# avadakadabra0909/geth-sharding

Hardware: AMD Instinct MI355X
Metric: ecrecover sigs/sec + Keccak collation GB/s (higher is better)
Workload: dtype u32; 1 GPU; 1M-signature secp256k1 ecrecover + Keccak-256 address derivation per GPU (BASELINE.json configs[1]); signatures_per_gpu=1048576, parallelism=shard-partitioned x1, batches_in_flight=2

## Files before the change

geth-sharding_amd/csrc/fe9_asm.cuh:

```cuda
#pragma once
#include <stdint.h>
namespace gsv {
__device__ __forceinline__ void fe9_mul_full(uint32_t r[9], const uint32_t a[9], const uint32_t b[9]) {
    uint64_t sd;
    uint32_t k31264 = 31264u, k256 = 256u, k977 = 977u, k8192 = 8192u;
    asm("v_mad_u64_u32 v[2:3], %9, %11, %27, 0\n\tv_mad_u64_u32 v[2:3], %9, %12, %26, v[2:3]\n\tv_mad_u64_u32 v[2:3], %9, %13, %25, v[2:3]\n\tv_mad_u64_u32 v[2:3], %9, %14, %24, v[2:3]\n\tv_mad_u64_u32 v[2:3], %9, %15, %23, v[2:3]\n\tv_mad_u64_u32 v[2:3], %9, %16, %22, v[2:3]\n\tv_mad_u64_u32 v[2:3], %9, %17, %21, v[2:3]\n\tv_mad_u64_u32 v[2:3], %9, %18, %20, v[2:3]\n\tv_mad_u64_u32 v[6:7], %9, v3, 8, 0\n\tv_mad_u64_u32 v[6:7], %9, %12, %27, v[6:7]\n\tv_mad_u64_u32 v[6:7], %9, %13, %26, v[6:7]\n\tv_mad_u64_u32 v[6:7], %9, %14, %25, v[6:7]\n\tv_mad_u64_u32 v[6:7], %9, %15, %24, v[6:7]\n\tv_mad_u64_u32 v[6:7], %9, %16, %23, v[6:7]\n\tv_mad_u64_u32 v[6:7], %9, %17, %22, v[6:7]\n\tv_mad_u64_u32 v[6:7], %9, %18, %21, v[6:7]\n\tv_mad_u64_u32 v[8:9], %9, v7, 8, 0\n\tv_mad_u64_u32 v[8:9], %9, %13, %27, v[8:9]\n\tv_mad_u64_u32 v[8:9], %9, %14, %26, v[8:9]\n\tv_mad_u64_u32 v[8:9], %9, %15, %25, v[8:9]\n\tv_mad_u64_u32 v[8:9], %9, %16, %24, v[8:9]\n\tv_mad_u64_u32 v[8:9], %9, %17, %23, v[8:9]\n\tv_mad_u64_u32 v[8:9], %9, %18, %22, v[8:9]\n\tv_mad_u64_u32 v[10:11], %9, v9, 8, 0\n\tv_mad_u64_u32 v[10:11], %9, %14, %27, v[10:11]\n\tv_mad_u64_u32 v[10:11], %9, %15, %26, v[10:11]\n\tv_mad_u64_u32 v[10:11], %9, %16, %25, v[10:11]\n\tv_mad_u64_u32 v[10:11], %9, %17, %24, v[10:11]\n\tv_mad_u64_u32 v[10:11], %9, %18, %23, v[10:11]\n\tv_mad_u64_u32 v[12:13], %9, v11, 8, 0\n\tv_mad_u64_u32 v[12:13], %9, %15, %27, v[12:13]\n\tv_mad_u64_u32 v[12:13], %9, %16, %26, v[12:13]\n\tv_mad_u64_u32 v[12:13], %9, %17, %25, v[12:13]\n\tv_mad_u64_u32 v[12:13], %9, %18, %24, v[12:13]\n\tv_mad_u64_u32 v[14:15], %9, v13, 8, 0\n\tv_mad_u64_u32 v[14:15], %9, %16, %27, v[14:15]\n\tv_mad_u64_u32 v[14:15], %9, %17, %26, v[14:15]\n\tv_mad_u64_u32 v[14:15], %9, %18, %25, v[14:15]\n\tv_mad_u64_u32 v[16:17], %9, v15, 8, 0\n\tv_mad_u64_u32 v[16:17], %9, %17, %27, v[16:17]\n\tv_mad_u64_u32 v[16:17], %9, %18, %26, v[16:17]\n\tv_mad_u64_u32 v[18:19], %9, v17, 8, 0\n\tv_mad_u64_u32 v[18:19], %9, %18, %27, v[18:19]\n\tv_lshlrev_b32 v3, 3, v19\n\tv_mad_u64_u32 v[4:5], %9, %10, %19, 0\n\tv_mad_u64_u32 v[4:5], %9, v2, %28, v[4:5]\n\tv_and_b32_e32 %0, 0x1fffffff, v4\n\tv_lshrrev_b64 v[4:5], 29, v[4:5]\n\tv_mad_u64_u32 v[4:5], %9, %10, %20, v[4:5]\n\tv_mad_u64_u32 v[4:5], %9, %11, %19, v[4:5]\n\tv_mad_u64_u32 v[4:5], %9, v6, %28, v[4:5]\n\tv_mad_u64_u32 v[4:5], %9, v2, %29, v[4:5]\n\tv_and_b32_e32 %1, 0x1fffffff, v4\n\tv_lshrrev_b64 v[4:5], 29, v[4:5]\n\tv_mad_u64_u32 v[4:5], %9, %10, %21, v[4:5]\n\tv_mad_u64_u32 v[4:5], %9, %11, %20, v[4:5]\n\tv_mad_u64_u32 v[4:5], %9, %12, %19, v[4:5]\n\tv_mad_u64_u32 v[4:5], %9, v8, %28, v[4:5]\n\tv_mad_u64_u32 v[4:5], %9, v6, %29, v[4:5]\n\tv_and_b32_e32 %2, 0x1fffffff, v4\n\tv_lshrrev_b64 v[4:5], 29, v[4:5]\n\tv_mad_u64_u32 v[4:5], %9, %10, %22, v[4:5]\n\tv_mad_u64_u32 v[4:5], %9, %11, %21, v[4:5]\n\tv_mad_u64_u32 v[4:5], %9, %12, %20, v[4:5]\n\tv_mad_u64_u32 v[4:5], %9, %13, %19, v[4:5]\n\tv_mad_u64_u32 v[4:5], %9, v10, %28, v[4:5]\n\tv_mad_u64_u32 v[4:5], %9, v8, %29, v[4:5]\n\tv_and_b32_e32 %3, 0x1fffffff, v4\n\tv_lshrrev_b64 v[4:5], 29, v[4:5]\n\tv_mad_u64_u32 v[4:5], %9, %10, %23, v[4:5]\n\tv_mad_u64_u32 v[4:5], %9, %11, %22, v[4:5]\n\tv_mad_u64_u32 v[4:5], %9, %12, %21, v[4:5]\n\tv_mad_u64_u32 v[4:5], %9, %13, %20, v[4:5]\n\tv_mad_u64_u32 v[4:5], %9, %14, %19, v[4:5]\n\tv_mad_u64_u32 v[4:5], %9, v12, %28, v[4:5]\n\tv_mad_u64_u32 v[4:5], %9, v10, %29, v[4:5]\n\tv_and_b32_e32 %4, 0x1fffffff, v4\n\tv_lshrrev_b64 v[4:5], 29, v[4:5]\n\tv_mad_u64_u32 v[4:5], %9, %10, %24, v[4:5]\n\tv_mad_u64_u32 v[4:5], %9, %11, %23, v[4:5]\n\tv_mad_u64_u32 v[4:5], %9, %12, %22, v[4:5]\n\tv_mad_u64_u32 v[4:5], %9, %13, %21, v[4:5]\n\tv_mad_u64_u32 v[4:5], %9, %14, %20, v[4:5]\n\tv_mad_u64_u32 v[4:5], %9, %15, %19, v[4:5]\n\tv_mad_u64_u32 v[4:5], %9, v14, %28, v[4:5]\n\tv_mad_u64_u32 v[4:5], %9, v12, %29, v[4:5]\n\tv_and_b32_e32 %5, 0x1fffffff, v4\n\tv_lshrrev_b64 v[4:5], 29, v[4:5]\n\tv_mad_u64_u32 v[4:5], %9, %10, %25, v[4:5]\n\tv_mad_u64_u32 v[4:5], %9, %11, %24, v[4:5]\n\tv_mad_u64_u32 v[4:5], %9, %12, %23, v[4:5]\n\tv_mad_u64_u32 v[4:5], %9, %13, %22, v[4:5]\n\tv_mad_u64_u32 v[4:5], %9, %14, %21, v[4:5]\n\tv_mad_u64_u32 v[4:5], %9, %15, %20, v[4:5]\n\tv_mad_u64_u32 v[4:5], %9, %16, %19, v[4:5]\n\tv_mad_u64_u32 v[4:5], %9, v16, %28, v[4:5]\n\tv_mad_u64_u32 v[4:5], %9, v14, %29, v[4:5]\n\tv_and_b32_e32 %6, 0x1fffffff, v4\n\tv_lshrrev_b64 v[4:5], 29, v[4:5]\n\tv_mad_u64_u32 v[4:5], %9, %10, %26, v[4:5]\n\tv_mad_u64_u32 v[4:5], %9, %11, %25, v[4:5]\n\tv_mad_u64_u32 v[4:5], %9, %12, %24, v[4:5]\n\tv_mad_u64_u32 v[4:5], %9, %13, %23, v[4:5]\n\tv_mad_u64_u32 v[4:5], %9, %14, %22, v[4:5]\n\tv_mad_u64_u32 v[4:5], %9, %15, %21, v[4:5]\n\tv_mad_u64_u32 v[4:5], %9, %16, %20, v[4:5]\n\tv_mad_u64_u32 v[4:5], %9, %17, %19, v[4:5]\n\tv_mad_u64_u32 v[4:5], %9, v18, %28, v[4:5]\n\tv_mad_u64_u32 v[4:5], %9, v16, %29, v[4:5]\n\tv_and_b32_e32 %7, 0x1fffffff, v4\n\tv_lshrrev_b64 v[4:5], 29, v[4:5]\n\tv_mad_u64_u32 v[4:5], %9, %10, %27, v[4:5]\n\tv_mad_u64_u32 v[4:5], %9, %11, %26, v[4:5]\n\tv_mad_u64_u32 v[4:5], %9, %12, %25, v[4:5]\n\tv_mad_u64_u32 v[4:5], %9, %13, %24, v[4:5]\n\tv_mad_u64_u32 v[4:5], %9, %14, %23, v[4:5]\n\tv_mad_u64_u32 v[4:5], %9, %15, %22, v[4:5]\n\tv_mad_u64_u32 v[4:5], %9, %16, %21, v[4:5]\n\tv_mad_u64_u32 v[4:5], %9, %17, %20, v[4:5]\n\tv_mad_u64_u32 v[4:5], %9, %18, %19, v[4:5]\n\tv_mad_u64_u32 v[4:5], %9, v3, %28, v[4:5]\n\tv_mad_u64_u32 v[4:5], %9, v18, %29, v[4:5]\n\tv_and_b32_e32 %8, 0xffffff, v4\n\tv_lshrrev_b64 v[4:5], 24, v[4:5]\n\tv_mad_u64_u32 v[6:7], %9, v3, %31, v[4:5]\n\tv_mov_b32 v5, 0\n\tv_mov_b32 v4, %0\n\tv_mad_u64_u32 v[4:5], %9, v6, %30, v[4:5]\n\tv_mad_u32_u24 v5, v7, %30, v5\n\tv_and_b32_e32 %0, 0x1fffffff, v4\n\tv_lshrrev_b64 v[4:5], 29, v[4:5]\n\tv_lshl_add_u64 v[4:5], v[6:7], 3, v[4:5]\n\tv_mad_u64_u32 v[4:5], %9, %1, 1, v[4:5]\n\tv_and_b32_e32 %1, 0x1fffffff, v4\n\tv_alignbit_b32 v6, v5, v4, 29\n\tv_add_u32 %2, %2, v6"
        : "=&v"(r[0]), "=&v"(r[1]), "=&v"(r[2]), "=&v"(r[3]), "=&v"(r[4]), "=&v"(r[5]), "=&v"(r[6]), "=&v"(r[7]), "=&v"(r[8]), "=&s"(sd)
        : "v"(a[0]), "v"(a[1]), "v"(a[2]), "v"(a[3]), "v"(a[4]), "v"(a[5]), "v"(a[6]), "v"(a[7]), "v"(a[8]), "v"(b[0]), "v"(b[1]), "v"(b[2]), "v"(b[3]), "v"(b[4]), "v"(b[5]), "v"(b[6]), "v"(b[7]), "v"(b[8]), "s"(k31264), "s"(k256), "s"(k977), "s"(k8192)
        : "v2", "v3", "v4", "v5", "v6", "v7", "v8", "v9", "v10", "v11", "v12", "v13", "v14", "v15", "v16", "v17", "v18", "v19");
}
__device__ __forceinline__ void fe9_sqr_full(uint32_t r[9], const uint32_t a[9], const uint32_t b[9]) {
    uint64_t sd;
    uint32_t k31264 = 31264u, k256 = 256u, k977 = 977u, k8192 = 8192u;
    asm("v_mad_u64_u32 v[2:3], %9, %11, %27, 0\n\tv_mad_u64_u32 v[2:3], %9, %12, %26, v[2:3]\n\tv_mad_u64_u32 v[2:3], %9, %13, %25, v[2:3]\n\tv_mad_u64_u32 v[2:3], %9, %14, %24, v[2:3]\n\tv_mad_u64_u32 v[6:7], %9, v3, 8, 0\n\tv_mad_u64_u32 v[6:7], %9, %12, %27, v[6:7]\n\tv_mad_u64_u32 v[6:7], %9, %13, %26, v[6:7]\n\tv_mad_u64_u32 v[6:7], %9, %14, %25, v[6:7]\n\tv_mad_u64_u32 v[6:7], %9, %15, %15, v[6:7]\n\tv_mad_u64_u32 v[8:9], %9, v7, 8, 0\n\tv_mad_u64_u32 v[8:9], %9, %13, %27, v[8:9]\n\tv_mad_u64_u32 v[8:9], %9, %14, %26, v[8:9]\n\tv_mad_u64_u32 v[8:9], %9, %15, %25, v[8:9]\n\tv_mad_u64_u32 v[10:11], %9, v9, 8, 0\n\tv_mad_u64_u32 v[10:11], %9, %14, %27, v[10:11]\n\tv_mad_u64_u32 v[10:11], %9, %15, %26, v[10:11]\n\tv_mad_u64_u32 v[10:11], %9, %16, %16, v[10:11]\n\tv_mad_u64_u32 v[12:13], %9, v11, 8, 0\n\tv_mad_u64_u32 v[12:13], %9, %15, %27, v[12:13]\n\tv_mad_u64_u32 v[12:13], %9, %16, %26, v[12:13]\n\tv_mad_u64_u32 v[14:15], %9, v13, 8, 0\n\tv_mad_u64_u32 v[14:15], %9, %16, %27, v[14:15]\n\tv_mad_u64_u32 v[14:15], %9, %17, %17, v[14:15]\n\tv_mad_u64_u32 v[16:17], %9, v15, 8, 0\n\tv_mad_u64_u32 v[16:17], %9, %17, %27, v[16:17]\n\tv_mad_u64_u32 v[18:19], %9, v17, 8, 0\n\tv_mad_u64_u32 v[18:19], %9, %18, %18, v[18:19]\n\tv_lshlrev_b32 v3, 3, v19\n\tv_mad_u64_u32 v[4:5], %9, %10, %10, 0\n\tv_mad_u64_u32 v[4:5], %9, v2, %28, v[4:5]\n\tv_and_b32_e32 %0, 0x1fffffff, v4\n\tv_lshrrev_b64 v[4:5], 29, v[4:5]\n\tv_mad_u64_u32 v[4:5], %9, %10, %20, v[4:5]\n\tv_mad_u64_u32 v[4:5], %9, v6, %28, v[4:5]\n\tv_mad_u64_u32 v[4:5], %9, v2, %29, v[4:5]\n\tv_and_b32_e32 %1, 0x1fffffff, v4\n\tv_lshrrev_b64 v[4:5], 29, v[4:5]\n\tv_mad_u64_u32 v[4:5], %9, %10, %21, v[4:5]\n\tv_mad_u64_u32 v[4:5], %9, %11, %11, v[4:5]\n\tv_mad_u64_u32 v[4:5], %9, v8, %28, v[4:5]\n\tv_mad_u64_u32 v[4:5], %9, v6, %29, v[4:5]\n\tv_and_b32_e32 %2, 0x1fffffff, v4\n\tv_lshrrev_b64 v[4:5], 29, v[4:5]\n\tv_mad_u64_u32 v[4:5], %9, %10, %22, v[4:5]\n\tv_mad_u64_u32 v[4:5], %9, %11, %21, v[4:5]\n\tv_mad_u64_u32 v[4:5], %9, v10, %28, v[4:5]\n\tv_mad_u64_u32 v[4:5], %9, v8, %29, v[4:5]\n\tv_and_b32_e32 %3, 0x1fffffff, v4\n\tv_lshrrev_b64 v[4:5], 29, v[4:5]\n\tv_mad_u64_u32 v[4:5], %9, %10, %23, v[4:5]\n\tv_mad_u64_u32 v[4:5], %9, %11, %22, v[4:5]\n\tv_mad_u64_u32 v[4:5], %9, %12, %12, v[4:5]\n\tv_mad_u64_u32 v[4:5], %9, v12, %28, v[4:5]\n\tv_mad_u64_u32 v[4:5], %9, v10, %29, v[4:5]\n\tv_and_b32_e32 %4, 0x1fffffff, v4\n\tv_lshrrev_b64 v[4:5], 29, v[4:5]\n\tv_mad_u64_u32 v[4:5], %9, %10, %24, v[4:5]\n\tv_mad_u64_u32 v[4:5], %9, %11, %23, v[4:5]\n\tv_mad_u64_u32 v[4:5], %9, %12, %22, v[4:5]\n\tv_mad_u64_u32 v[4:5], %9, v14, %28, v[4:5]\n\tv_mad_u64_u32 v[4:5], %9, v12, %29, v[4:5]\n\tv_and_b32_e32 %5, 0x1fffffff, v4\n\tv_lshrrev_b64 v[4:5], 29, v[4:5]\n\tv_mad_u64_u32 v[4:5], %9, %10, %25, v[4:5]\n\tv_mad_u64_u32 v[4:5], %9, %11, %24, v[4:5]\n\tv_mad_u64_u32 v[4:5], %9, %12, %23, v[4:5]\n\tv_mad_u64_u32 v[4:5], %9, %13, %13, v[4:5]\n\tv_mad_u64_u32 v[4:5], %9, v16, %28, v[4:5]\n\tv_mad_u64_u32 v[4:5], %9, v14, %29, v[4:5]\n\tv_and_b32_e32 %6, 0x1fffffff, v4\n\tv_lshrrev_b64 v[4:5], 29, v[4:5]\n\tv_mad_u64_u32 v[4:5], %9, %10, %26, v[4:5]\n\tv_mad_u64_u32 v[4:5], %9, %11, %25, v[4:5]\n\tv_mad_u64_u32 v[4:5], %9, %12, %24, v[4:5]\n\tv_mad_u64_u32 v[4:5], %9, %13, %23, v[4:5]\n\tv_mad_u64_u32 v[4:5], %9, v18, %28, v[4:5]\n\tv_mad_u64_u32 v[4:5], %9, v16, %29, v[4:5]\n\tv_and_b32_e32 %7, 0x1fffffff, v4\n\tv_lshrrev_b64 v[4:5], 29, v[4:5]\n\tv_mad_u64_u32 v[4:5], %9, %10, %27, v[4:5]\n\tv_mad_u64_u32 v[4:5], %9, %11, %26, v[4:5]\n\tv_mad_u64_u32 v[4:5], %9, %12, %25, v[4:5]\n\tv_mad_u64_u32 v[4:5], %9, %13, %24, v[4:5]\n\tv_mad_u64_u32 v[4:5], %9, %14, %14, v[4:5]\n\tv_mad_u64_u32 v[4:5], %9, v3, %28, v[4:5]\n\tv_mad_u64_u32 v[4:5], %9, v18, %29, v[4:5]\n\tv_and_b32_e32 %8, 0xffffff, v4\n\tv_lshrrev_b64 v[4:5], 24, v[4:5]\n\tv_mad_u64_u32 v[6:7], %9, v3, %31, v[4:5]\n\tv_mov_b32 v5, 0\n\tv_mov_b32 v4, %0\n\tv_mad_u64_u32 v[4:5], %9, v6, %30, v[4:5]\n\tv_mad_u32_u24 v5, v7, %30, v5\n\tv_and_b32_e32 %0, 0x1fffffff, v4\n\tv_lshrrev_b64 v[4:5], 29, v[4:5]\n\tv_lshl_add_u64 v[4:5], v[6:7], 3, v[4:5]\n\tv_mad_u64_u32 v[4:5], %9, %1, 1, v[4:5]\n\tv_and_b32_e32 %1, 0x1fffffff, v4\n\tv_alignbit_b32 v6, v5, v4, 29\n\tv_add_u32 %2, %2, v6"
        : "=&v"(r[0]), "=&v"(r[1]), "=&v"(r[2]), "=&v"(r[3]), "=&v"(r[4]), "=&v"(r[5]), "=&v"(r[6]), "=&v"(r[7]), "=&v"(r[8]), "=&s"(sd)
        : "v"(a[0]), "v"(a[1]), "v"(a[2]), "v"(a[3]), "v"(a[4]), "v"(a[5]), "v"(a[6]), "v"(a[7]), "v"(a[8]), "v"(b[0]), "v"(b[1]), "v"(b[2]), "v"(b[3]), "v"(b[4]), "v"(b[5]), "v"(b[6]), "v"(b[7]), "v"(b[8]), "s"(k31264), "s"(k256), "s"(k977), "s"(k8192)
        : "v2", "v3", "v4", "v5", "v6", "v7", "v8", "v9", "v10", "v11", "v12", "v13", "v14", "v15", "v16", "v17", "v18", "v19");
}
__device__ __forceinline__ void fe9_mul_add_full(uint32_t r[9], const uint32_t a[9], const uint32_t b[9], const uint32_t c[9]) {
    uint64_t sd;
    uint32_t k31264 = 31264u, k256 = 256u, k977 = 977u, k8192 = 8192u;
    asm("v_mad_u64_u32 v[2:3], %9, %11, %27, 0\n\tv_mad_u64_u32 v[2:3], %9, %12, %26, v[2:3]\n\tv_mad_u64_u32 v[2:3], %9, %13, %25, v[2:3]\n\tv_mad_u64_u32 v[2:3], %9, %14, %24, v[2:3]\n\tv_mad_u64_u32 v[2:3], %9, %15, %23, v[2:3]\n\tv_mad_u64_u32 v[2:3], %9, %16, %22, v[2:3]\n\tv_mad_u64_u32 v[2:3], %9, %17, %21, v[2:3]\n\tv_mad_u64_u32 v[2:3], %9, %18, %20, v[2:3]\n\tv_mad_u64_u32 v[6:7], %9, v3, 8, 0\n\tv_mad_u64_u32 v[6:7], %9, %12, %27, v[6:7]\n\tv_mad_u64_u32 v[6:7], %9, %13, %26, v[6:7]\n\tv_mad_u64_u32 v[6:7], %9, %14, %25, v[6:7]\n\tv_mad_u64_u32 v[6:7], %9, %15, %24, v[6:7]\n\tv_mad_u64_u32 v[6:7], %9, %16, %23, v[6:7]\n\tv_mad_u64_u32 v[6:7], %9, %17, %22, v[6:7]\n\tv_mad_u64_u32 v[6:7], %9, %18, %21, v[6:7]\n\tv_mad_u64_u32 v[8:9], %9, v7, 8, 0\n\tv_mad_u64_u32 v[8:9], %9, %13, %27, v[8:9]\n\tv_mad_u64_u32 v[8:9], %9, %14, %26, v[8:9]\n\tv_mad_u64_u32 v[8:9], %9, %15, %25, v[8:9]\n\tv_mad_u64_u32 v[8:9], %9, %16, %24, v[8:9]\n\tv_mad_u64_u32 v[8:9], %9, %17, %23, v[8:9]\n\tv_mad_u64_u32 v[8:9], %9, %18, %22, v[8:9]\n\tv_mad_u64_u32 v[10:11], %9, v9, 8, 0\n\tv_mad_u64_u32 v[10:11], %9, %14, %27, v[10:11]\n\tv_mad_u64_u32 v[10:11], %9, %15, %26, v[10:11]\n\tv_mad_u64_u32 v[10:11], %9, %16, %25, v[10:11]\n\tv_mad_u64_u32 v[10:11], %9, %17, %24, v[10:11]\n\tv_mad_u64_u32 v[10:11], %9, %18, %23, v[10:11]\n\tv_mad_u64_u32 v[12:13], %9, v11, 8, 0\n\tv_mad_u64_u32 v[12:13], %9, %15, %27, v[12:13]\n\tv_mad_u64_u32 v[12:13], %9, %16, %26, v[12:13]\n\tv_mad_u64_u32 v[12:13], %9, %17, %25, v[12:13]\n\tv_mad_u64_u32 v[12:13], %9, %18, %24, v[12:13]\n\tv_mad_u64_u32 v[14:15], %9, v13, 8, 0\n\tv_mad_u64_u32 v[14:15], %9, %16, %27, v[14:15]\n\tv_mad_u64_u32 v[14:15], %9, %17, %26, v[14:15]\n\tv_mad_u64_u32 v[14:15], %9, %18, %25, v[14:15]\n\tv_mad_u64_u32 v[16:17], %9, v15, 8, 0\n\tv_mad_u64_u32 v[16:17], %9, %17, %27, v[16:17]\n\tv_mad_u64_u32 v[16:17], %9, %18, %26, v[16:17]\n\tv_mad_u64_u32 v[18:19], %9, v17, 8, 0\n\tv_mad_u64_u32 v[18:19], %9, %18, %27, v[18:19]\n\tv_lshlrev_b32 v3, 3, v19\n\tv_mad_u64_u32 v[4:5], %9, %32, 1, 0\n\tv_mad_u64_u32 v[4:5], %9, %10, %19, v[4:5]\n\tv_mad_u64_u32 v[4:5], %9, v2, %28, v[4:5]\n\tv_and_b32_e32 %0, 0x1fffffff, v4\n\tv_lshrrev_b64 v[4:5], 29, v[4:5]\n\tv_mad_u64_u32 v[4:5], %9, %33, 1, v[4:5]\n\tv_mad_u64_u32 v[4:5], %9, %10, %20, v[4:5]\n\tv_mad_u64_u32 v[4:5], %9, %11, %19, v[4:5]\n\tv_mad_u64_u32 v[4:5], %9, v6, %28, v[4:5]\n\tv_mad_u64_u32 v[4:5], %9, v2, %29, v[4:5]\n\tv_and_b32_e32 %1, 0x1fffffff, v4\n\tv_lshrrev_b64 v[4:5], 29, v[4:5]\n\tv_mad_u64_u32 v[4:5], %9, %34, 1, v[4:5]\n\tv_mad_u64_u32 v[4:5], %9, %10, %21, v[4:5]\n\tv_mad_u64_u32 v[4:5], %9, %11, %20, v[4:5]\n\tv_mad_u64_u32 v[4:5], %9, %12, %19, v[4:5]\n\tv_mad_u64_u32 v[4:5], %9, v8, %28, v[4:5]\n\tv_mad_u64_u32 v[4:5], %9, v6, %29, v[4:5]\n\tv_and_b32_e32 %2, 0x1fffffff, v4\n\tv_lshrrev_b64 v[4:5], 29, v[4:5]\n\tv_mad_u64_u32 v[4:5], %9, %35, 1, v[4:5]\n\tv_mad_u64_u32 v[4:5], %9, %10, %22, v[4:5]\n\tv_mad_u64_u32 v[4:5], %9, %11, %21, v[4:5]\n\tv_mad_u64_u32 v[4:5], %9, %12, %20, v[4:5]\n\tv_mad_u64_u32 v[4:5], %9, %13, %19, v[4:5]\n\tv_mad_u64_u32 v[4:5], %9, v10, %28, v[4:5]\n\tv_mad_u64_u32 v[4:5], %9, v8, %29, v[4:5]\n\tv_and_b32_e32 %3, 0x1fffffff, v4\n\tv_lshrrev_b64 v[4:5], 29, v[4:5]\n\tv_mad_u64_u32 v[4:5], %9, %36, 1, v[4:5]\n\tv_mad_u64_u32 v[4:5], %9, %10, %23, v[4:5]\n\tv_mad_u64_u32 v[4:5], %9, %11, %22, v[4:5]\n\tv_mad_u64_u32 v[4:5], %9, %12, %21, v[4:5]\n\tv_mad_u64_u32 v[4:5], %9, %13, %20, v[4:5]\n\tv_mad_u64_u32 v[4:5], %9, %14, %19, v[4:5]\n\tv_mad_u64_u32 v[4:5], %9, v12, %28, v[4:5]\n\tv_mad_u64_u32 v[4:5], %9, v10, %29, v[4:5]\n\tv_and_b32_e32 %4, 0x1fffffff, v4\n\tv_lshrrev_b64 v[4:5], 29, v[4:5]\n\tv_mad_u64_u32 v[4:5], %9, %37, 1, v[4:5]\n\tv_mad_u64_u32 v[4:5], %9, %10, %24, v[4:5]\n\tv_mad_u64_u32 v[4:5], %9, %11, %23, v[4:5]\n\tv_mad_u64_u32 v[4:5], %9, %12, %22, v[4:5]\n\tv_mad_u64_u32 v[4:5], %9, %13, %21, v[4:5]\n\tv_mad_u64_u32 v[4:5], %9, %14, %20, v[4:5]\n\tv_mad_u64_u32 v[4:5], %9, %15, %19, v[4:5]\n\tv_mad_u64_u32 v[4:5], %9, v14, %28, v[4:5]\n\tv_mad_u64_u32 v[4:5], %9, v12, %29, v[4:5]\n\tv_and_b32_e32 %5, 0x1fffffff, v4\n\tv_lshrrev_b64 v[4:5], 29, v[4:5]\n\tv_mad_u64_u32 v[4:5], %9, %38, 1, v[4:5]\n\tv_mad_u64_u32 v[4:5], %9, %10, %25, v[4:5]\n\tv_mad_u64_u32 v[4:5], %9, %11, %24, v[4:5]\n\tv_mad_u64_u32 v[4:5], %9, %12, %23, v[4:5]\n\tv_mad_u64_u32 v[4:5], %9, %13, %22, v[4:5]\n\tv_mad_u64_u32 v[4:5], %9, %14, %21, v[4:5]\n\tv_mad_u64_u32 v[4:5], %9, %15, %20, v[4:5]\n\tv_mad_u64_u32 v[4:5], %9, %16, %19, v[4:5]\n\tv_mad_u64_u32 v[4:5], %9, v16, %28, v[4:5]\n\tv_mad_u64_u32 v[4:5], %9, v14, %29, v[4:5]\n\tv_and_b32_e32 %6, 0x1fffffff, v4\n\tv_lshrrev_b64 v[4:5], 29, v[4:5]\n\tv_mad_u64_u32 v[4:5], %9, %39, 1, v[4:5]\n\tv_mad_u64_u32 v[4:5], %9, %10, %26, v[4:5]\n\tv_mad_u64_u32 v[4:5], %9, %11, %25, v[4:5]\n\tv_mad_u64_u32 v[4:5], %9, %12, %24, v[4:5]\n\tv_mad_u64_u32 v[4:5], %9, %13, %23, v[4:5]\n\tv_mad_u64_u32 v[4:5], %9, %14, %22, v[4:5]\n\tv_mad_u64_u32 v[4:5], %9, %15, %21, v[4:5]\n\tv_mad_u64_u32 v[4:5], %9, %16, %20, v[4:5]\n\tv_mad_u64_u32 v[4:5], %9, %17, %19, v[4:5]\n\tv_mad_u64_u32 v[4:5], %9, v18, %28, v[4:5]\n\tv_mad_u64_u32 v[4:5], %9, v16, %29, v[4:5]\n\tv_and_b32_e32 %7, 0x1fffffff, v4\n\tv_lshrrev_b64 v[4:5], 29, v[4:5]\n\tv_mad_u64_u32 v[4:5], %9, %40, 1, v[4:5]\n\tv_mad_u64_u32 v[4:5], %9, %10, %27, v[4:5]\n\tv_mad_u64_u32 v[4:5], %9, %11, %26, v[4:5]\n\tv_mad_u64_u32 v[4:5], %9, %12, %25, v[4:5]\n\tv_mad_u64_u32 v[4:5], %9, %13, %24, v[4:5]\n\tv_mad_u64_u32 v[4:5], %9, %14, %23, v[4:5]\n\tv_mad_u64_u32 v[4:5], %9, %15, %22, v[4:5]\n\tv_mad_u64_u32 v[4:5], %9, %16, %21, v[4:5]\n\tv_mad_u64_u32 v[4:5], %9, %17, %20, v[4:5]\n\tv_mad_u64_u32 v[4:5], %9, %18, %19, v[4:5]\n\tv_mad_u64_u32 v[4:5], %9, v3, %28, v[4:5]\n\tv_mad_u64_u32 v[4:5], %9, v18, %29, v[4:5]\n\tv_and_b32_e32 %8, 0xffffff, v4\n\tv_lshrrev_b64 v[4:5], 24, v[4:5]\n\tv_mad_u64_u32 v[6:7], %9, v3, %31, v[4:5]\n\tv_mov_b32 v5, 0\n\tv_mov_b32 v4, %0\n\tv_mad_u64_u32 v[4:5], %9, v6, %30, v[4:5]\n\tv_mad_u32_u24 v5, v7, %30, v5\n\tv_and_b32_e32 %0, 0x1fffffff, v4\n\tv_lshrrev_b64 v[4:5], 29, v[4:5]\n\tv_lshl_add_u64 v[4:5], v[6:7], 3, v[4:5]\n\tv_mad_u64_u32 v[4:5], %9, %1, 1, v[4:5]\n\tv_and_b32_e32 %1, 0x1fffffff, v4\n\tv_alignbit_b32 v6, v5, v4, 29\n\tv_add_u32 %2, %2, v6"
        : "=&v"(r[0]), "=&v"(r[1]), "=&v"(r[2]), "=&v"(r[3]), "=&v"(r[4]), "=&v"(r[5]), "=&v"(r[6]), "=&v"(r[7]), "=&v"(r[8]), "=&s"(sd)
        : "v"(a[0]), "v"(a[1]), "v"(a[2]), "v"(a[3]), "v"(a[4]), "v"(a[5]), "v"(a[6]), "v"(a[7]), "v"(a[8]), "v"(b[0]), "v"(b[1]), "v"(b[2]), "v"(b[3]), "v"(b[4]), "v"(b[5]), "v"(b[6]), "v"(b[7]), "v"(b[8]), "s"(k31264), "s"(k256), "s"(k977), "s"(k8192), "v"(c[0]), "v"(c[1]), "v"(c[2]), "v"(c[3]), "v"(c[4]), "v"(c[5]), "v"(c[6]), "v"(c[7]), "v"(c[8])
        : "v2", "v3", "v4", "v5", "v6", "v7", "v8", "v9", "v10", "v11", "v12", "v13", "v14", "v15", "v16", "v17", "v18", "v19");
}
__device__ __forceinline__ void fe9_sqr_add_full(uint32_t r[9], const uint32_t a[9], const uint32_t b[9], const uint32_t c[9]) {
    uint64_t sd;
    uint32_t k31264 = 31264u, k256 = 256u, k977 = 977u, k8192 = 8192u;
    asm("v_mad_u64_u32 v[2:3], %9, %11, %27, 0\n\tv_mad_u64_u32 v[2:3], %9, %12, %26, v[2:3]\n\tv_mad_u64_u32 v[2:3], %9, %13, %25, v[2:3]\n\tv_mad_u64_u32 v[2:3], %9, %14, %24, v[2:3]\n\tv_mad_u64_u32 v[6:7], %9, v3, 8, 0\n\tv_mad_u64_u32 v[6:7], %9, %12, %27, v[6:7]\n\tv_mad_u64_u32 v[6:7], %9, %13, %26, v[6:7]\n\tv_mad_u64_u32 v[6:7], %9, %14, %25, v[6:7]\n\tv_mad_u64_u32 v[6:7], %9, %15, %15, v[6:7]\n\tv_mad_u64_u32 v[8:9], %9, v7, 8, 0\n\tv_mad_u64_u32 v[8:9], %9, %13, %27, v[8:9]\n\tv_mad_u64_u32 v[8:9], %9, %14, %26, v[8:9]\n\tv_mad_u64_u32 v[8:9], %9, %15, %25, v[8:9]\n\tv_mad_u64_u32 v[10:11], %9, v9, 8, 0\n\tv_mad_u64_u32 v[10:11], %9, %14, %27, v[10:11]\n\tv_mad_u64_u32 v[10:11], %9, %15, %26, v[10:11]\n\tv_mad_u64_u32 v[10:11], %9, %16, %16, v[10:11]\n\tv_mad_u64_u32 v[12:13], %9, v11, 8, 0\n\tv_mad_u64_u32 v[12:13], %9, %15, %27, v[12:13]\n\tv_mad_u64_u32 v[12:13], %9, %16, %26, v[12:13]\n\tv_mad_u64_u32 v[14:15], %9, v13, 8, 0\n\tv_mad_u64_u32 v[14:15], %9, %16, %27, v[14:15]\n\tv_mad_u64_u32 v[14:15], %9, %17, %17, v[14:15]\n\tv_mad_u64_u32 v[16:17], %9, v15, 8, 0\n\tv_mad_u64_u32 v[16:17], %9, %17, %27, v[16:17]\n\tv_mad_u64_u32 v[18:19], %9, v17, 8, 0\n\tv_mad_u64_u32 v[18:19], %9, %18, %18, v[18:19]\n\tv_lshlrev_b32 v3, 3, v19\n\tv_mad_u64_u32 v[4:5], %9, %32, 1, 0\n\tv_mad_u64_u32 v[4:5], %9, %10, %10, v[4:5]\n\tv_mad_u64_u32 v[4:5], %9, v2, %28, v[4:5]\n\tv_and_b32_e32 %0, 0x1fffffff, v4\n\tv_lshrrev_b64 v[4:5], 29, v[4:5]\n\tv_mad_u64_u32 v[4:5], %9, %33, 1, v[4:5]\n\tv_mad_u64_u32 v[4:5], %9, %10, %20, v[4:5]\n\tv_mad_u64_u32 v[4:5], %9, v6, %28, v[4:5]\n\tv_mad_u64_u32 v[4:5], %9, v2, %29, v[4:5]\n\tv_and_b32_e32 %1, 0x1fffffff, v4\n\tv_lshrrev_b64 v[4:5], 29, v[4:5]\n\tv_mad_u64_u32 v[4:5], %9, %34, 1, v[4:5]\n\tv_mad_u64_u32 v[4:5], %9, %10, %21, v[4:5]\n\tv_mad_u64_u32 v[4:5], %9, %11, %11, v[4:5]\n\tv_mad_u64_u32 v[4:5], %9, v8, %28, v[4:5]\n\tv_mad_u64_u32 v[4:5], %9, v6, %29, v[4:5]\n\tv_and_b32_e32 %2, 0x1fffffff, v4\n\tv_lshrrev_b64 v[4:5], 29, v[4:5]\n\tv_mad_u64_u32 v[4:5], %9, %35, 1, v[4:5]\n\tv_mad_u64_u32 v[4:5], %9, %10, %22, v[4:5]\n\tv_mad_u64_u32 v[4:5], %9, %11, %21, v[4:5]\n\tv_mad_u64_u32 v[4:5], %9, v10, %28, v[4:5]\n\tv_mad_u64_u32 v[4:5], %9, v8, %29, v[4:5]\n\tv_and_b32_e32 %3, 0x1fffffff, v4\n\tv_lshrrev_b64 v[4:5], 29, v[4:5]\n\tv_mad_u64_u32 v[4:5], %9, %36, 1, v[4:5]\n\tv_mad_u64_u32 v[4:5], %9, %10, %23, v[4:5]\n\tv_mad_u64_u32 v[4:5], %9, %11, %22, v[4:5]\n\tv_mad_u64_u32 v[4:5], %9, %12, %12, v[4:5]\n\tv_mad_u64_u32 v[4:5], %9, v12, %28, v[4:5]\n\tv_mad_u64_u32 v[4:5], %9, v10, %29, v[4:5]\n\tv_and_b32_e32 %4, 0x1fffffff, v4\n\tv_lshrrev_b64 v[4:5], 29, v[4:5]\n\tv_mad_u64_u32 v[4:5], %9, %37, 1, v[4:5]\n\tv_mad_u64_u32 v[4:5], %9, %10, %24, v[4:5]\n\tv_mad_u64_u32 v[4:5], %9, %11, %23, v[4:5]\n\tv_mad_u64_u32 v[4:5], %9, %12, %22, v[4:5]\n\tv_mad_u64_u32 v[4:5], %9, v14, %28, v[4:5]\n\tv_mad_u64_u32 v[4:5], %9, v12, %29, v[4:5]\n\tv_and_b32_e32 %5, 0x1fffffff, v4\n\tv_lshrrev_b64 v[4:5], 29, v[4:5]\n\tv_mad_u64_u32 v[4:5], %9, %38, 1, v[4:5]\n\tv_mad_u64_u32 v[4:5], %9, %10, %25, v[4:5]\n\tv_mad_u64_u32 v[4:5], %9, %11, %24, v[4:5]\n\tv_mad_u64_u32 v[4:5], %9, %12, %23, v[4:5]\n\tv_mad_u64_u32 v[4:5], %9, %13, %13, v[4:5]\n\tv_mad_u64_u32 v[4:5], %9, v16, %28, v[4:5]\n\tv_mad_u64_u32 v[4:5], %9, v14, %29, v[4:5]\n\tv_and_b32_e32 %6, 0x1fffffff, v4\n\tv_lshrrev_b64 v[4:5], 29, v[4:5]\n\tv_mad_u64_u32 v[4:5], %9, %39, 1, v[4:5]\n\tv_mad_u64_u32 v[4:5], %9, %10, %26, v[4:5]\n\tv_mad_u64_u32 v[4:5], %9, %11, %25, v[4:5]\n\tv_mad_u64_u32 v[4:5], %9, %12, %24, v[4:5]\n\tv_mad_u64_u32 v[4:5], %9, %13, %23, v[4:5]\n\tv_mad_u64_u32 v[4:5], %9, v18, %28, v[4:5]\n\tv_mad_u64_u32 v[4:5], %9, v16, %29, v[4:5]\n\tv_and_b32_e32 %7, 0x1fffffff, v4\n\tv_lshrrev_b64 v[4:5], 29, v[4:5]\n\tv_mad_u64_u32 v[4:5], %9, %40, 1, v[4:5]\n\tv_mad_u64_u32 v[4:5], %9, %10, %27, v[4:5]\n\tv_mad_u64_u32 v[4:5], %9, %11, %26, v[4:5]\n\tv_mad_u64_u32 v[4:5], %9, %12, %25, v[4:5]\n\tv_mad_u64_u32 v[4:5], %9, %13, %24, v[4:5]\n\tv_mad_u64_u32 v[4:5], %9, %14, %14, v[4:5]\n\tv_mad_u64_u32 v[4:5], %9, v3, %28, v[4:5]\n\tv_mad_u64_u32 v[4:5], %9, v18, %29, v[4:5]\n\tv_and_b32_e32 %8, 0xffffff, v4\n\tv_lshrrev_b64 v[4:5], 24, v[4:5]\n\tv_mad_u64_u32 v[6:7], %9, v3, %31, v[4:5]\n\tv_mov_b32 v5, 0\n\tv_mov_b32 v4, %0\n\tv_mad_u64_u32 v[4:5], %9, v6, %30, v[4:5]\n\tv_mad_u32_u24 v5, v7, %30, v5\n\tv_and_b32_e32 %0, 0x1fffffff, v4\n\tv_lshrrev_b64 v[4:5], 29, v[4:5]\n\tv_lshl_add_u64 v[4:5], v[6:7], 3, v[4:5]\n\tv_mad_u64_u32 v[4:5], %9, %1, 1, v[4:5]\n\tv_and_b32_e32 %1, 0x1fffffff, v4\n\tv_alignbit_b32 v6, v5, v4, 29\n\tv_add_u32 %2, %2, v6"
        : "=&v"(r[0]), "=&v"(r[1]), "=&v"(r[2]), "=&v"(r[3]), "=&v"(r[4]), "=&v"(r[5]), "=&v"(r[6]), "=&v"(r[7]), "=&v"(r[8]), "=&s"(sd)
        : "v"(a[0]), "v"(a[1]), "v"(a[2]), "v"(a[3]), "v"(a[4]), "v"(a[5]), "v"(a[6]), "v"(a[7]), "v"(a[8]), "v"(b[0]), "v"(b[1]), "v"(b[2]), "v"(b[3]), "v"(b[4]), "v"(b[5]), "v"(b[6]), "v"(b[7]), "v"(b[8]), "s"(k31264), "s"(k256), "s"(k977), "s"(k8192), "v"(c[0]), "v"(c[1]), "v"(c[2]), "v"(c[3]), "v"(c[4]), "v"(c[5]), "v"(c[6]), "v"(c[7]), "v"(c[8])
        : "v2", "v3", "v4", "v5", "v6", "v7", "v8", "v9", "v10", "v11", "v12", "v13", "v14", "v15", "v16", "v17", "v18", "v19");
}
__device__ __forceinline__ void fe9_dot_full(uint32_t r[9], const uint32_t a[9], const uint32_t b[9], const uint32_t c[9], const uint32_t d[9]) {
    uint64_t sd;
    uint32_t k31264 = 31264u, k256 = 256u, k977 = 977u, k8192 = 8192u;
    asm("v_mad_u64_u32 v[2:3], %9, %11, %27, 0\n\tv_mad_u64_u32 v[2:3], %9, %12, %26, v[2:3]\n\tv_mad_u64_u32 v[2:3], %9, %13, %25, v[2:3]\n\tv_mad_u64_u32 v[2:3], %9, %14, %24, v[2:3]\n\tv_mad_u64_u32 v[2:3], %9, %15, %23, v[2:3]\n\tv_mad_u64_u32 v[2:3], %9, %16, %22, v[2:3]\n\tv_mad_u64_u32 v[2:3], %9, %17, %21, v[2:3]\n\tv_mad_u64_u32 v[2:3], %9, %18, %20, v[2:3]\n\tv_mad_u64_u32 v[2:3], %9, %33, %49, v[2:3]\n\tv_mad_u64_u32 v[2:3], %9, %34, %48, v[2:3]\n\tv_mad_u64_u32 v[2:3], %9, %35, %47, v[2:3]\n\tv_mad_u64_u32 v[2:3], %9, %36, %46, v[2:3]\n\tv_mad_u64_u32 v[2:3], %9, %37, %45, v[2:3]\n\tv_mad_u64_u32 v[2:3], %9, %38, %44, v[2:3]\n\tv_mad_u64_u32 v[2:3], %9, %39, %43, v[2:3]\n\tv_mad_u64_u32 v[2:3], %9, %40, %42, v[2:3]\n\tv_mad_u64_u32 v[6:7], %9, v3, 8, 0\n\tv_mad_u64_u32 v[6:7], %9, %12, %27, v[6:7]\n\tv_mad_u64_u32 v[6:7], %9, %13, %26, v[6:7]\n\tv_mad_u64_u32 v[6:7], %9, %14, %25, v[6:7]\n\tv_mad_u64_u32 v[6:7], %9, %15, %24, v[6:7]\n\tv_mad_u64_u32 v[6:7], %9, %16, %23, v[6:7]\n\tv_mad_u64_u32 v[6:7], %9, %17, %22, v[6:7]\n\tv_mad_u64_u32 v[6:7], %9, %18, %21, v[6:7]\n\tv_mad_u64_u32 v[6:7], %9, %34, %49, v[6:7]\n\tv_mad_u64_u32 v[6:7], %9, %35, %48, v[6:7]\n\tv_mad_u64_u32 v[6:7], %9, %36, %47, v[6:7]\n\tv_mad_u64_u32 v[6:7], %9, %37, %46, v[6:7]\n\tv_mad_u64_u32 v[6:7], %9, %38, %45, v[6:7]\n\tv_mad_u64_u32 v[6:7], %9, %39, %44, v[6:7]\n\tv_mad_u64_u32 v[6:7], %9, %40, %43, v[6:7]\n\tv_mad_u64_u32 v[8:9], %9, v7, 8, 0\n\tv_mad_u64_u32 v[8:9], %9, %13, %27, v[8:9]\n\tv_mad_u64_u32 v[8:9], %9, %14, %26, v[8:9]\n\tv_mad_u64_u32 v[8:9], %9, %15, %25, v[8:9]\n\tv_mad_u64_u32 v[8:9], %9, %16, %24, v[8:9]\n\tv_mad_u64_u32 v[8:9], %9, %17, %23, v[8:9]\n\tv_mad_u64_u32 v[8:9], %9, %18, %22, v[8:9]\n\tv_mad_u64_u32 v[8:9], %9, %35, %49, v[8:9]\n\tv_mad_u64_u32 v[8:9], %9, %36, %48, v[8:9]\n\tv_mad_u64_u32 v[8:9], %9, %37, %47, v[8:9]\n\tv_mad_u64_u32 v[8:9], %9, %38, %46, v[8:9]\n\tv_mad_u64_u32 v[8:9], %9, %39, %45, v[8:9]\n\tv_mad_u64_u32 v[8:9], %9, %40, %44, v[8:9]\n\tv_mad_u64_u32 v[10:11], %9, v9, 8, 0\n\tv_mad_u64_u32 v[10:11], %9, %14, %27, v[10:11]\n\tv_mad_u64_u32 v[10:11], %9, %15, %26, v[10:11]\n\tv_mad_u64_u32 v[10:11], %9, %16, %25, v[10:11]\n\tv_mad_u64_u32 v[10:11], %9, %17, %24, v[10:11]\n\tv_mad_u64_u32 v[10:11], %9, %18, %23, v[10:11]\n\tv_mad_u64_u32 v[10:11], %9, %36, %49, v[10:11]\n\tv_mad_u64_u32 v[10:11], %9, %37, %48, v[10:11]\n\tv_mad_u64_u32 v[10:11], %9, %38, %47, v[10:11]\n\tv_mad_u64_u32 v[10:11], %9, %39, %46, v[10:11]\n\tv_mad_u64_u32 v[10:11], %9, %40, %45, v[10:11]\n\tv_mad_u64_u32 v[12:13], %9, v11, 8, 0\n\tv_mad_u64_u32 v[12:13], %9, %15, %27, v[12:13]\n\tv_mad_u64_u32 v[12:13], %9, %16, %26, v[12:13]\n\tv_mad_u64_u32 v[12:13], %9, %17, %25, v[12:13]\n\tv_mad_u64_u32 v[12:13], %9, %18, %24, v[12:13]\n\tv_mad_u64_u32 v[12:13], %9, %37, %49, v[12:13]\n\tv_mad_u64_u32 v[12:13], %9, %38, %48, v[12:13]\n\tv_mad_u64_u32 v[12:13], %9, %39, %47, v[12:13]\n\tv_mad_u64_u32 v[12:13], %9, %40, %46, v[12:13]\n\tv_mad_u64_u32 v[14:15], %9, v13, 8, 0\n\tv_mad_u64_u32 v[14:15], %9, %16, %27, v[14:15]\n\tv_mad_u64_u32 v[14:15], %9, %17, %26, v[14:15]\n\tv_mad_u64_u32 v[14:15], %9, %18, %25, v[14:15]\n\tv_mad_u64_u32 v[14:15], %9, %38, %49, v[14:15]\n\tv_mad_u64_u32 v[14:15], %9, %39, %48, v[14:15]\n\tv_mad_u64_u32 v[14:15], %9, %40, %47, v[14:15]\n\tv_mad_u64_u32 v[16:17], %9, v15, 8, 0\n\tv_mad_u64_u32 v[16:17], %9, %17, %27, v[16:17]\n\tv_mad_u64_u32 v[16:17], %9, %18, %26, v[16:17]\n\tv_mad_u64_u32 v[16:17], %9, %39, %49, v[16:17]\n\tv_mad_u64_u32 v[16:17], %9, %40, %48, v[16:17]\n\tv_mad_u64_u32 v[18:19], %9, v17, 8, 0\n\tv_mad_u64_u32 v[18:19], %9, %18, %27, v[18:19]\n\tv_mad_u64_u32 v[18:19], %9, %40, %49, v[18:19]\n\tv_lshlrev_b32 v3, 3, v19\n\tv_mad_u64_u32 v[4:5], %9, %10, %19, 0\n\tv_mad_u64_u32 v[4:5], %9, %32, %41, v[4:5]\n\tv_mad_u64_u32 v[4:5], %9, v2, %28, v[4:5]\n\tv_and_b32_e32 %0, 0x1fffffff, v4\n\tv_lshrrev_b64 v[4:5], 29, v[4:5]\n\tv_mad_u64_u32 v[4:5], %9, %10, %20, v[4:5]\n\tv_mad_u64_u32 v[4:5], %9, %11, %19, v[4:5]\n\tv_mad_u64_u32 v[4:5], %9, %32, %42, v[4:5]\n\tv_mad_u64_u32 v[4:5], %9, %33, %41, v[4:5]\n\tv_mad_u64_u32 v[4:5], %9, v6, %28, v[4:5]\n\tv_mad_u64_u32 v[4:5], %9, v2, %29, v[4:5]\n\tv_and_b32_e32 %1, 0x1fffffff, v4\n\tv_lshrrev_b64 v[4:5], 29, v[4:5]\n\tv_mad_u64_u32 v[4:5], %9, %10, %21, v[4:5]\n\tv_mad_u64_u32 v[4:5], %9, %11, %20, v[4:5]\n\tv_mad_u64_u32 v[4:5], %9, %12, %19, v[4:5]\n\tv_mad_u64_u32 v[4:5], %9, %32, %43, v[4:5]\n\tv_mad_u64_u32 v[4:5], %9, %33, %42, v[4:5]\n\tv_mad_u64_u32 v[4:5], %9, %34, %41, v[4:5]\n\tv_mad_u64_u32 v[4:5], %9, v8, %28, v[4:5]\n\tv_mad_u64_u32 v[4:5], %9, v6, %29, v[4:5]\n\tv_and_b32_e32 %2, 0x1fffffff, v4\n\tv_lshrrev_b64 v[4:5], 29, v[4:5]\n\tv_mad_u64_u32 v[4:5], %9, %10, %22, v[4:5]\n\tv_mad_u64_u32 v[4:5], %9, %11, %21, v[4:5]\n\tv_mad_u64_u32 v[4:5], %9, %12, %20, v[4:5]\n\tv_mad_u64_u32 v[4:5], %9, %13, %19, v[4:5]\n\tv_mad_u64_u32 v[4:5], %9, %32, %44, v[4:5]\n\tv_mad_u64_u32 v[4:5], %9, %33, %43, v[4:5]\n\tv_mad_u64_u32 v[4:5], %9, %34, %42, v[4:5]\n\tv_mad_u64_u32 v[4:5], %9, %35, %41, v[4:5]\n\tv_mad_u64_u32 v[4:5], %9, v10, %28, v[4:5]\n\tv_mad_u64_u32 v[4:5], %9, v8, %29, v[4:5]\n\tv_and_b32_e32 %3, 0x1fffffff, v4\n\tv_lshrrev_b64 v[4:5], 29, v[4:5]\n\tv_mad_u64_u32 v[4:5], %9, %10, %23, v[4:5]\n\tv_mad_u64_u32 v[4:5], %9, %11, %22, v[4:5]\n\tv_mad_u64_u32 v[4:5], %9, %12, %21, v[4:5]\n\tv_mad_u64_u32 v[4:5], %9, %13, %20, v[4:5]\n\tv_mad_u64_u32 v[4:5], %9, %14, %19, v[4:5]\n\tv_mad_u64_u32 v[4:5], %9, %32, %45, v[4:5]\n\tv_mad_u64_u32 v[4:5], %9, %33, %44, v[4:5]\n\tv_mad_u64_u32 v[4:5], %9, %34, %43, v[4:5]\n\tv_mad_u64_u32 v[4:5], %9, %35, %42, v[4:5]\n\tv_mad_u64_u32 v[4:5], %9, %36, %41, v[4:5]\n\tv_mad_u64_u32 v[4:5], %9, v12, %28, v[4:5]\n\tv_mad_u64_u32 v[4:5], %9, v10, %29, v[4:5]\n\tv_and_b32_e32 %4, 0x1fffffff, v4\n\tv_lshrrev_b64 v[4:5], 29, v[4:5]\n\tv_mad_u64_u32 v[4:5], %9, %10, %24, v[4:5]\n\tv_mad_u64_u32 v[4:5], %9, %11, %23, v[4:5]\n\tv_mad_u64_u32 v[4:5], %9, %12, %22, v[4:5]\n\tv_mad_u64_u32 v[4:5], %9, %13, %21, v[4:5]\n\tv_mad_u64_u32 v[4:5], %9, %14, %20, v[4:5]\n\tv_mad_u64_u32 v[4:5], %9, %15, %19, v[4:5]\n\tv_mad_u64_u32 v[4:5], %9, %32, %46, v[4:5]\n\tv_mad_u64_u32 v[4:5], %9, %33, %45, v[4:5]\n\tv_mad_u64_u32 v[4:5], %9, %34, %44, v[4:5]\n\tv_mad_u64_u32 v[4:5], %9, %35, %43, v[4:5]\n\tv_mad_u64_u32 v[4:5], %9, %36, %42, v[4:5]\n\tv_mad_u64_u32 v[4:5], %9, %37, %41, v[4:5]\n\tv_mad_u64_u32 v[4:5], %9, v14, %28, v[4:5]\n\tv_mad_u64_u32 v[4:5], %9, v12, %29, v[4:5]\n\tv_and_b32_e32 %5, 0x1fffffff, v4\n\tv_lshrrev_b64 v[4:5], 29, v[4:5]\n\tv_mad_u64_u32 v[4:5], %9, %10, %25, v[4:5]\n\tv_mad_u64_u32 v[4:5], %9, %11, %24, v[4:5]\n\tv_mad_u64_u32 v[4:5], %9, %12, %23, v[4:5]\n\tv_mad_u64_u32 v[4:5], %9, %13, %22, v[4:5]\n\tv_mad_u64_u32 v[4:5], %9, %14, %21, v[4:5]\n\tv_mad_u64_u32 v[4:5], %9, %15, %20, v[4:5]\n\tv_mad_u64_u32 v[4:5], %9, %16, %19, v[4:5]\n\tv_mad_u64_u32 v[4:5], %9, %32, %47, v[4:5]\n\tv_mad_u64_u32 v[4:5], %9, %33, %46, v[4:5]\n\tv_mad_u64_u32 v[4:5], %9, %34, %45, v[4:5]\n\tv_mad_u64_u32 v[4:5], %9, %35, %44, v[4:5]\n\tv_mad_u64_u32 v[4:5], %9, %36, %43, v[4:5]\n\tv_mad_u64_u32 v[4:5], %9, %37, %42, v[4:5]\n\tv_mad_u64_u32 v[4:5], %9, %38, %41, v[4:5]\n\tv_mad_u64_u32 v[4:5], %9, v16, %28, v[4:5]\n\tv_mad_u64_u32 v[4:5], %9, v14, %29, v[4:5]\n\tv_and_b32_e32 %6, 0x1fffffff, v4\n\tv_lshrrev_b64 v[4:5], 29, v[4:5]\n\tv_mad_u64_u32 v[4:5], %9, %10, %26, v[4:5]\n\tv_mad_u64_u32 v[4:5], %9, %11, %25, v[4:5]\n\tv_mad_u64_u32 v[4:5], %9, %12, %24, v[4:5]\n\tv_mad_u64_u32 v[4:5], %9, %13, %23, v[4:5]\n\tv_mad_u64_u32 v[4:5], %9, %14, %22, v[4:5]\n\tv_mad_u64_u32 v[4:5], %9, %15, %21, v[4:5]\n\tv_mad_u64_u32 v[4:5], %9, %16, %20, v[4:5]\n\tv_mad_u64_u32 v[4:5], %9, %17, %19, v[4:5]\n\tv_mad_u64_u32 v[4:5], %9, %32, %48, v[4:5]\n\tv_mad_u64_u32 v[4:5], %9, %33, %47, v[4:5]\n\tv_mad_u64_u32 v[4:5], %9, %34, %46, v[4:5]\n\tv_mad_u64_u32 v[4:5], %9, %35, %45, v[4:5]\n\tv_mad_u64_u32 v[4:5], %9, %36, %44, v[4:5]\n\tv_mad_u64_u32 v[4:5], %9, %37, %43, v[4:5]\n\tv_mad_u64_u32 v[4:5], %9, %38, %42, v[4:5]\n\tv_mad_u64_u32 v[4:5], %9, %39, %41, v[4:5]\n\tv_mad_u64_u32 v[4:5], %9, v18, %28, v[4:5]\n\tv_mad_u64_u32 v[4:5], %9, v16, %29, v[4:5]\n\tv_and_b32_e32 %7, 0x1fffffff, v4\n\tv_lshrrev_b64 v[4:5], 29, v[4:5]\n\tv_mad_u64_u32 v[4:5], %9, %10, %27, v[4:5]\n\tv_mad_u64_u32 v[4:5], %9, %11, %26, v[4:5]\n\tv_mad_u64_u32 v[4:5], %9, %12, %25, v[4:5]\n\tv_mad_u64_u32 v[4:5], %9, %13, %24, v[4:5]\n\tv_mad_u64_u32 v[4:5], %9, %14, %23, v[4:5]\n\tv_mad_u64_u32 v[4:5], %9, %15, %22, v[4:5]\n\tv_mad_u64_u32 v[4:5], %9, %16, %21, v[4:5]\n\tv_mad_u64_u32 v[4:5], %9, %17, %20, v[4:5]\n\tv_mad_u64_u32 v[4:5], %9, %18, %19, v[4:5]\n\tv_mad_u64_u32 v[4:5], %9, %32, %49, v[4:5]\n\tv_mad_u64_u32 v[4:5], %9, %33, %48, v[4:5]\n\tv_mad_u64_u32 v[4:5], %9, %34, %47, v[4:5]\n\tv_mad_u64_u32 v[4:5], %9, %35, %46, v[4:5]\n\tv_mad_u64_u32 v[4:5], %9, %36, %45, v[4:5]\n\tv_mad_u64_u32 v[4:5], %9, %37, %44, v[4:5]\n\tv_mad_u64_u32 v[4:5], %9, %38, %43, v[4:5]\n\tv_mad_u64_u32 v[4:5], %9, %39, %42, v[4:5]\n\tv_mad_u64_u32 v[4:5], %9, %40, %41, v[4:5]\n\tv_mad_u64_u32 v[4:5], %9, v3, %28, v[4:5]\n\tv_mad_u64_u32 v[4:5], %9, v18, %29, v[4:5]\n\tv_and_b32_e32 %8, 0xffffff, v4\n\tv_lshrrev_b64 v[4:5], 24, v[4:5]\n\tv_mad_u64_u32 v[6:7], %9, v3, %31, v[4:5]\n\tv_mov_b32 v5, 0\n\tv_mov_b32 v4, %0\n\tv_mad_u64_u32 v[4:5], %9, v6, %30, v[4:5]\n\tv_mad_u32_u24 v5, v7, %30, v5\n\tv_and_b32_e32 %0, 0x1fffffff, v4\n\tv_lshrrev_b64 v[4:5], 29, v[4:5]\n\tv_lshl_add_u64 v[4:5], v[6:7], 3, v[4:5]\n\tv_mad_u64_u32 v[4:5], %9, %1, 1, v[4:5]\n\tv_and_b32_e32 %1, 0x1fffffff, v4\n\tv_alignbit_b32 v6, v5, v4, 29\n\tv_add_u32 %2, %2, v6"
        : "=&v"(r[0]), "=&v"(r[1]), "=&v"(r[2]), "=&v"(r[3]), "=&v"(r[4]), "=&v"(r[5]), "=&v"(r[6]), "=&v"(r[7]), "=&v"(r[8]), "=&s"(sd)
        : "v"(a[0]), "v"(a[1]), "v"(a[2]), "v"(a[3]), "v"(a[4]), "v"(a[5]), "v"(a[6]), "v"(a[7]), "v"(a[8]), "v"(b[0]), "v"(b[1]), "v"(b[2]), "v"(b[3]), "v"(b[4]), "v"(b[5]), "v"(b[6]), "v"(b[7]), "v"(b[8]), "s"(k31264), "s"(k256), "s"(k977), "s"(k8192), "v"(c[0]), "v"(c[1]), "v"(c[2]), "v"(c[3]), "v"(c[4]), "v"(c[5]), "v"(c[6]), "v"(c[7]), "v"(c[8]), "v"(d[0]), "v"(d[1]), "v"(d[2]), "v"(d[3]), "v"(d[4]), "v"(d[5]), "v"(d[6]), "v"(d[7]), "v"(d[8])
        : "v2", "v3", "v4", "v5", "v6", "v7", "v8", "v9", "v10", "v11", "v12", "v13", "v14", "v15", "v16", "v17", "v18", "v19");
}
}
```

geth-sharding_amd/csrc/opcount.cuh:

```cuda
#pragma once

namespace gsv {
enum OpKind : int {
    OPC_FE_MUL = 0,
    OPC_FE_SQR = 1,
    OPC_SC_MUL = 2,
    OPC_SC_SQR = 3,
    OPC_BN_MUL = 4,
    OPC_MODINV = 5,
    OPC_BN_REDC = 6,
    OPC_FE_DOT = 7,
    OPC_N = 8
};
}

#if defined(GSV_OPCOUNT) && defined(__HIPCC__)
#include <hip/hip_runtime.h>
static __device__ unsigned long long gsv_opc_counts[gsv::OPC_N];
__device__ __forceinline__ void gsv_opc(int k) {
    unsigned long long m = __ballot(1);
    if ((int)__lane_id() == __ffsll((long long)m) - 1) atomicAdd(&gsv_opc_counts[k], (unsigned long long)__popcll(m));
}
#define GSV_OPC(k) gsv_opc(k)
#define GSV_OPCOUNT_READER(name)                                                                       \
    extern "C" int gsv_opcount_##name(unsigned long long* out, int reset) {                            \
        if (hipDeviceSynchronize() != hipSuccess) return -1;                                           \
        if (hipMemcpyFromSymbol(out, HIP_SYMBOL(gsv_opc_counts), sizeof(gsv_opc_counts)) != hipSuccess) \
            return -1;                                                                                 \
        if (reset) {                                                                                   \
            unsigned long long z[gsv::OPC_N] = {0};                                                    \
            if (hipMemcpyToSymbol(HIP_SYMBOL(gsv_opc_counts), z, sizeof(z)) != hipSuccess) return -1;  \
        }                                                                                              \
        return 0;                                                                                      \
    }
#else
#define GSV_OPC(k) ((void)0)
#define GSV_OPCOUNT_READER(name)
#endif
```

geth-sharding_amd/csrc/recover_dev.cuh:

```cuda
#pragma once
#include "gsv_internal.h"
#include "keccak_dev.cuh"
#include "secp256k1_dev.cuh"
namespace gsv { struct gej9; __device__ void gej9_dbl_rare(gej9& o, const gej9& p); }
#define GEJ9_DBL_RARE(o, p) gej9_dbl_rare(o, p)
#include "secp256k1_fe9.cuh"
#include "modinv30.cuh"

namespace gsv {

__device__ constexpr uint32_t BETA[8] = {0x719501EEu, 0xC1396C28u, 0x12F58995u, 0x9CF04975u,
                                         0xAC3434E9u, 0x6E64479Eu, 0x657C0710u, 0x7AE96A2Bu};
__device__ constexpr uint32_t MINUS_LAMBDA[8] = {0xB51283CFu, 0xE0CFC810u, 0x8EC739C2u, 0xA880B9FCu,
                                                 0x77ED9BA4u, 0x5AD9E3FDu, 0x3FA3CF1Fu, 0xAC9C52B3u};
__device__ constexpr uint32_t MINUS_B1[8] = {0x0ABFE4C3u, 0x6F547FA9u, 0x010E8828u, 0xE4437ED6u,
                                             0u, 0u, 0u, 0u};
__device__ constexpr uint32_t MINUS_B2[8] = {0x3DB1562Cu, 0xD765CDA8u, 0x0774346Du, 0x8A280AC5u,
                                             0xFFFFFFFEu, 0xFFFFFFFFu, 0xFFFFFFFFu, 0xFFFFFFFFu};
__device__ constexpr uint32_t GLV_G1[8] = {0xEB153DABu, 0x90E49284u, 0x6BCDE86Cu, 0xD221A7D4u,
                                           0x00003086u, 0u, 0u, 0u};
__device__ constexpr uint32_t GLV_G2[8] = {0xE4C42212u, 0x7FA90ABFu, 0x88286F54u, 0x7ED6010Eu,
                                           0x0000E443u, 0u, 0u, 0u};
__device__ constexpr uint32_t GX[8] = {0x16F81798u, 0x59F2815Bu, 0x2DCE28D9u, 0x029BFCDBu,
                                       0xCE870B07u, 0x55A06295u, 0xF9DCBBACu, 0x79BE667Eu};
__device__ constexpr uint32_t GY[8] = {0xFB10D4B8u, 0x9C47D08Fu, 0xA6855419u, 0xFD17B448u,
                                       0x0E1108A8u, 0x5DA4FBFCu, 0x26A3C465u, 0x483ADA77u};
__device__ constexpr uint32_t P_MINUS_N[8] = {0x2FC9BAEEu, 0x402DA172u, 0x50B75FC4u, 0x45512319u,
                                              0x00000001u, 0u, 0u, 0u};
__device__ constexpr uint32_t HALF_N[8] = {0x681B20A0u, 0xDFE92F46u, 0x57A4501Du, 0x5D576E73u,
                                           0xFFFFFFFFu, 0xFFFFFFFFu, 0xFFFFFFFFu, 0x7FFFFFFFu};

constexpr int GLV_W = 4;
constexpr int GLV_NT = 1 << (GLV_W - 1);
constexpr int GLV_DIGITS = (130 + GLV_W - 1) / GLV_W;
constexpr int DIG_SLOT = GLV_W <= 4 ? 4 : 8;
constexpr int DIG_PER_WORD = 32 / DIG_SLOT;
constexpr int DIG_WORDS = (GLV_DIGITS + DIG_PER_WORD - 1) / DIG_PER_WORD;
static_assert(GLV_W >= 3 && GLV_W <= 5, "GLV window width");
constexpr int GLV_LNT = 4;
static_assert(GLV_LNT <= GLV_NT, "LDS holds at most four entries at two waves per SIMD");
constexpr int GSV_LTAB_STRIDE = 256;
constexpr int GSV_LTAB_WORDS = 18 * GLV_LNT * GSV_LTAB_STRIDE;
#define GSV_ECR_WAVES 2
#define GSV_LTAB_DECL __shared__ uint32_t ltab[GSV_LTAB_WORDS]
#define GSV_LTAB_LANE (ltab + threadIdx.x)

GSV_DI void sc_from_const(sc& r, const uint32_t c[8]) {
#pragma unroll
    for (int i = 0; i < 8; i++) r.v[i] = c[i];
}

GSV_DI void sc_mul_shift272(sc& r, const sc& k, const uint32_t g[8]) {
    GSV_OPC(OPC_SC_MUL);
    uint32_t t[16];
    mul_8x8_fx(t, k.v, g);
#pragma unroll
    for (int i = 0; i < 7; i++) r.v[i] = (t[8 + i] >> 16) | (t[9 + i] << 16);
    r.v[7] = t[15] >> 16;
    uint64_t c = (uint64_t)r.v[0] + ((t[8] >> 15) & 1u);
    r.v[0] = lo32(c);
#pragma unroll
    for (int i = 1; i < 8; i++) {
        c = (uint64_t)r.v[i] + hi32(c);
        r.v[i] = lo32(c);
    }
}

GSV_DI void sc_split_lambda(sc& r1, sc& r2, const sc& k) {
    sc c1, c2, t;
    sc_mul_shift272(c1, k, GLV_G1);
    sc_mul_shift272(c2, k, GLV_G2);
    sc_from_const(t, MINUS_B1);
    sc_mul(c1, c1, t);
    sc_from_const(t, MINUS_B2);
    sc_mul(c2, c2, t);
    sc_add(r2, c1, c2);
    sc_from_const(t, MINUS_LAMBDA);
    sc_mul(r1, r2, t);
    sc_add(r1, r1, k);
}

GSV_DI bool sc_is_high(const sc& a) { return limbs_lt(HALF_N, a.v); }

GSV_DI void recode_glv(uint32_t dig[DIG_WORDS], uint32_t& skew, const sc& kin) {
    constexpr uint32_t MASK = (2u << GLV_W) - 1u;
    constexpr int32_t OFF = 1 << GLV_W;
    uint32_t k[5] = {kin.v[0], kin.v[1], kin.v[2], kin.v[3], kin.v[4]};
    skew = (k[0] & 1u) ^ 1u;
    uint64_t c = (uint64_t)k[0] + skew;
    k[0] = lo32(c);
#pragma unroll
    for (int i = 1; i < 5; i++) {
        c = (uint64_t)k[i] + hi32(c);
        k[i] = lo32(c);
    }
#pragma unroll
    for (int i = 0; i < DIG_WORDS; i++) dig[i] = 0;
#pragma unroll
    for (int i = 0; i < GLV_DIGITS; i++) {
        int32_t d;
        if (i < GLV_DIGITS - 1) d = (int32_t)(k[0] & MASK) - OFF;
        else d = (int32_t)(k[0] & MASK);
        uint32_t neg = d < 0 ? 1u : 0u;
        uint32_t mag = (uint32_t)(d < 0 ? -d : d);
        uint32_t code = (neg << (GLV_W - 1)) | ((mag - 1u) >> 1);
        dig[i / DIG_PER_WORD] |= code << ((i % DIG_PER_WORD) * DIG_SLOT);
        int64_t t = (int64_t)k[0] - d;
        uint32_t kk[5];
        kk[0] = (uint32_t)t;
        int64_t carry = t >> 32;
#pragma unroll
        for (int j = 1; j < 5; j++) {
            int64_t u = (int64_t)k[j] + carry;
            kk[j] = (uint32_t)u;
            carry = u >> 32;
        }
#pragma unroll
        for (int j = 0; j < 4; j++) k[j] = (kk[j] >> GLV_W) | (kk[j + 1] << (32 - GLV_W));
        k[4] = kk[4] >> GLV_W;
    }
}

GSV_DI void fe9_from_const(fe9& r, const uint32_t c[8]) {
    uint32_t w[8];
#pragma unroll
    for (int i = 0; i < 8; i++) w[i] = c[i];
    fe9_from_words(r, w);
}
GSV_DI void ge9_cmov(ge9& r, const ge9& a, bool f) {
    fe9_cmov(r.x, a.x, f);
    fe9_cmov(r.y, a.y, f);
}

typedef uint32_t gsv_v32 __attribute__((ext_vector_type(32)));
__device__ __noinline__ gsv_v32 gej9_dbl_ool(gsv_v32 in) {
    gej9 p, d;
#pragma unroll
    for (int i = 0; i < 9; i++) {
        p.x.v[i] = in[i];
        p.y.v[i] = in[9 + i];
        p.z.v[i] = in[18 + i];
    }
    gej9_dbl(d, p);
    gsv_v32 o;
#pragma unroll
    for (int i = 0; i < 9; i++) {
        o[i] = d.x.v[i];
        o[9 + i] = d.y.v[i];
        o[18 + i] = d.z.v[i];
    }
#pragma unroll
    for (int i = 27; i < 32; i++) o[i] = 0;
    return o;
}
__device__ void gej9_dbl_rare(gej9& o, const gej9& p) {
    gsv_v32 in;
#pragma unroll
    for (int i = 0; i < 9; i++) {
        in[i] = p.x.v[i];
        in[9 + i] = p.y.v[i];
        in[18 + i] = p.z.v[i];
    }
#pragma unroll
    for (int i = 27; i < 32; i++) in[i] = 0;
    gsv_v32 d = gej9_dbl_ool(in);
#pragma unroll
    for (int i = 0; i < 9; i++) {
        o.x.v[i] = d[i];
        o.y.v[i] = d[9 + i];
        o.z.v[i] = d[18 + i];
    }
}

GSV_DI void table_select9(ge9& out, const ge9 T[4], uint32_t idx) {
    out = T[0];
#pragma unroll
    for (int e = 1; e < 4; e++) ge9_cmov(out, T[e], idx == (uint32_t)e);
}
GSV_DI void table_select9_x(fe9& out, const fe9 X[4], uint32_t idx) {
    out = X[0];
#pragma unroll
    for (int e = 1; e < 4; e++) fe9_cmov(out, X[e], idx == (uint32_t)e);
}

constexpr int GTAB_ENTRY_U4 = GTAB_ENTRY_BYTES / 16;
GSV_DI void gtab_load(ge9& P, const uint4* e) {
    uint4 a = e[0], b = e[1], c = e[2], d = e[3], f = e[4];
    uint32_t w[20] = {a.x, a.y, a.z, a.w, b.x, b.y, b.z, b.w, c.x, c.y, c.z, c.w,
                      d.x, d.y, d.z, d.w, f.x, f.y, f.z, f.w};
#pragma unroll
    for (int i = 0; i < 9; i++) {
        P.x.v[i] = w[i];
        P.y.v[i] = w[9 + i];
    }
}

GSV_DI void comb_shift(uint32_t c[8]) {
#pragma unroll
    for (int i = 0; i < 7; i++) c[i] = __builtin_amdgcn_alignbit(c[i + 1], c[i], COMB_BITS);
    c[7] >>= COMB_BITS;
}
GSV_DI void comb_mul_g9(gej9& acc, bool& inf, const sc& u, const uint4* __restrict__ gtab) {
    constexpr uint32_t MASK = (1u << COMB_BITS) - 1u;
    uint32_t c[8] = {u.v[0], u.v[1], u.v[2], u.v[3], u.v[4], u.v[5], u.v[6], u.v[7]};
    ge9 Pn;
    const uint32_t d0 = c[0] & MASK;
    gtab_load(Pn, gtab + (size_t)d0 * GTAB_ENTRY_U4);
    acc.x = Pn.x;
    acc.y = Pn.y;
    fe9_set_u32(acc.z, 1);
    inf = d0 == 0;
    comb_shift(c);
    gtab_load(Pn, gtab + (((size_t)1 << COMB_BITS) + (c[0] & MASK)) * GTAB_ENTRY_U4);
#pragma unroll 1
    for (int w = 1; w < COMB_WINDOWS; w++) {
        uint32_t d = c[0] & MASK;
        ge9 P = Pn;
        if (w < COMB_WINDOWS - 1) {
            comb_shift(c);
            gtab_load(Pn, gtab + (((size_t)(w + 1) << COMB_BITS) + (c[0] & MASK)) * GTAB_ENTRY_U4);
        }
        gej9 t;
        bool tinf = inf;
        gej9_add_ge(t, tinf, acc, P);
        if (d != 0) {
            acc = t;
            inf = tinf;
        }
    }
}

GSV_DI void gej9_to_affine_words(fe& ax, fe& ay, const gej9& q) {
    fe9 zi, zi2, x, y;
    {
        fe9 z = q.z;
        fe9_normalize_full(z);
        uint32_t zw[8], iw[8];
        fe9_to_words(zw, z);
        modinv30_words(iw, zw, MI30_P);
        fe9_from_words(zi, iw);
    }
    fe9_sqr(zi2, zi);
    fe9_mul(x, q.x, zi2);
    fe9_mul(zi2, zi2, zi);
    fe9_mul(y, q.y, zi2);
    fe9_normalize_full(x);
    fe9_normalize_full(y);
    fe9_to_words(ax.v, x);
    fe9_to_words(ay.v, y);
}


GSV_DI bool recover_tail_twisted(fe& qx, fe& qy, const gej9& p1, bool p1inf, const gej9& p2, bool p2inf,
                                 const fe9& c, uint32_t par) {
    fe9 x3a, db, y3a, y3b, z;
    fe9 s1p, s2;
    bool exc;
    {
        fe9 z1z1, zz, z2z2, u1, h, t;
        fe9_sqr(z1z1, p1.z);
        fe9_sqr(zz, p2.z);
        fe9_mul(z2z2, c, zz);
        fe9_mul(u1, p1.x, z2z2);
        fe9_neg<1>(t, u1);
        fe9_mul_add(h, p2.x, z1z1, t);
        fe9_mul(s1p, p1.y, p2.z);
        fe9_mul(s1p, s1p, z2z2);
        fe9_mul(s2, p2.y, p1.z);
        fe9_mul(s2, s2, z1z1);
        exc = !p1inf && fe9_is_zero_weak(h);
        fe9 hh, hhh, v, cs1, a1;
        fe9_sqr(hh, h);
        fe9_mul(hhh, h, hh);
        fe9_mul(v, u1, hh);
        fe9_mul(cs1, c, s1p);
        fe9_negsum3<3>(t, hhh, v, v);
        fe9_sqr_add(a1, s2, t);
        fe9_mul_add(x3a, cs1, s1p, a1);
        fe9_mul(t, s2, s1p);
        fe9_add(db, t, t);
        fe9 da, ndb, e;
        fe9_sub<1>(da, v, x3a);
        fe9_neg<2>(ndb, db);
        fe9_dot(y3a, s2, da, cs1, ndb);
        fe9_add(e, da, hhh);
        fe9_normalize_weak(e);
        fe9_neg<1>(t, e);
        fe9_dot(y3b, s2, db, s1p, t);
        fe9_mul(t, p1.z, p2.z);
        fe9_mul(z, t, h);
    }
    if (FE9_ANY(exc)) {
        gej9 d;
        gej9_dbl(d, p2);
        fe9_cmov(x3a, d.x, exc);
        fe9_cmov(y3a, d.y, exc);
        fe9_cmov(z, d.z, exc);
        fe9_cmov(db, s1p, exc);
        fe9_cmov(y3b, s2, exc);
    }
    if (FE9_ANY(p1inf)) {
        fe9 zero;
        fe9_set_u32(zero, 0);
        fe9_cmov(x3a, p2.x, p1inf);
        fe9_cmov(y3a, p2.y, p1inf);
        fe9_cmov(z, p2.z, p1inf);
        fe9_cmov(db, zero, p1inf);
        fe9_cmov(y3b, zero, p1inf);
    }
    fe9 m, s0;
    bool ok;
    {
        fe9 z2, t, w;
        fe9_sqr(z2, z);
        fe9_sqr(t, z2);
        fe9_mul(t, t, c);
        fe9_pow_pm3_4(w, t);
        fe9_mul(m, w, z);
        fe9_mul(t, c, m);
        fe9_mul(s0, t, z);
        fe9_sqr(t, s0);
        fe9_normalize_full(t);
        fe9 cc = c;
        fe9_normalize_full(cc);
        ok = fe9_eq_canon(t, cc) && !p2inf;
    }
    fe9 s0n = s0;
    fe9_normalize_full(s0n);
    bool flip = (s0n.v[0] & 1u) != par;
    fe9 pb, qb;
    fe9_mul(pb, s0, db);
    fe9_mul(qb, s0, y3b);
    if (FE9_ANY(exc)) {
        fe9 a, b2;
        fe9_add(a, y3b, pb);
        fe9_sub<1>(b2, y3b, pb);
        fe9_cmov(b2, a, flip);
        bool rr0 = fe9_is_zero(b2);
        ok = ok && !(exc && !rr0);
        fe9 zero;
        fe9_set_u32(zero, 0);
        fe9_cmov(pb, zero, exc);
        fe9_cmov(qb, zero, exc);
    }
    fe9 m2, m3, n, xs, ys;
    fe9_sqr(m2, m);
    fe9_mul(m3, m2, m);
    fe9_neg<1>(n, pb);
    fe9_cmov(n, pb, flip);
    fe9_add(xs, x3a, n);
    fe9_neg<1>(n, y3a);
    fe9_cmov(n, y3a, !flip);
    fe9_add(ys, n, qb);
    fe9 x, y;
    fe9_mul(x, xs, m2);
    fe9_mul(y, ys, m3);
    fe9_normalize_full(x);
    fe9_normalize_full(y);
    fe9_to_words(qx.v, x);
    fe9_to_words(qy.v, y);
    return ok;
}

__device__ constexpr uint32_t GLV_V1A[8] = {0x9284EB15u, 0xE86C90E4u, 0xA7D46BCDu, 0x3086D221u, 0u, 0u, 0u, 0u};
__device__ constexpr uint32_t GLV_V1B[8] = {0xC5765C7Eu, 0x507DDEE3u, 0xAE3A1813u, 0xD66B5E10u,
                                            0xFFFFFFFDu, 0xFFFFFFFFu, 0xFFFFFFFFu, 0xFFFFFFFFu};
__device__ constexpr uint32_t GLV_V2A[8] = {0x9D44CFD8u, 0x57C1108Du, 0xA8E2F3F6u, 0x14CA50F7u, 1u, 0u, 0u, 0u};
__device__ constexpr uint32_t GLV_V3A[8] = {0x2FC9BAEDu, 0x402DA172u, 0x50B75FC4u, 0x45512319u, 1u, 0u, 0u, 0u};
__device__ constexpr uint32_t GLV_V3B[8] = {0x57FB4793u, 0x38EA6FC8u, 0x560E83E1u, 0x06F23032u,
                                            0xFFFFFFFEu, 0xFFFFFFFFu, 0xFFFFFFFFu, 0xFFFFFFFFu};
GSV_DI void glv_make_odd(sc& k1, sc& k2) {
    bool odd1 = ((k1.v[0] & 1u) != 0) != sc_is_high(k1);
    bool odd2 = ((k2.v[0] & 1u) != 0) != sc_is_high(k2);
    bool use1 = !odd1 && !odd2, use2 = odd1 && !odd2, use3 = !odd1 && odd2;
    sc A, B;
#pragma unroll
    for (int i = 0; i < 8; i++) {
        A.v[i] = use1 ? GLV_V1A[i] : use2 ? GLV_V2A[i] : use3 ? GLV_V3A[i] : 0u;
        B.v[i] = use1 ? GLV_V1B[i] : use2 ? GLV_V1A[i] : use3 ? GLV_V3B[i] : 0u;
    }
    sc_add(k1, k1, A);
    sc_add(k2, k2, B);
}

GSV_DI uint32_t recover_core(fe& qx, fe& qy, const uint32_t msg[8], const uint32_t r[8],
                             const uint32_t s[8], uint32_t recid, const uint4* __restrict__ gtab,
                             uint32_t* __restrict__ ltab) {
    bool ok = limbs_lt(r, SN) && limbs_lt(s, SN);
    sc rs, ss, m;
#pragma unroll
    for (int i = 0; i < 8; i++) {
        rs.v[i] = r[i];
        ss.v[i] = s[i];
    }
    ok = ok && !sc_is_zero(rs) && !sc_is_zero(ss);
    sc_cond_sub_n(m.v, msg, 0);

    fe9 x;
    {
        bool hi = (recid & 2u) != 0;
        ok = ok && (!hi || limbs_lt(r, P_MINUS_N));
        uint32_t xw[8];
        uint64_t c = 0;
#pragma unroll
        for (int i = 0; i < 8; i++) {
            c = (uint64_t)r[i] + (hi ? SN[i] : 0u) + hi32(c);
            xw[i] = lo32(c);
        }
        fe9_from_words(x, xw);
    }
    fe9 y, t;
    fe9 c;
    fe9_sqr(t, x);
    fe9_mul(c, t, x);
    c.v[0] += 7u;
    fe9_mul(t, c, x);
    fe9_sqr(y, c);
    x = t;
    sc rn, u1, u2;
    modinv30_words(rn.v, rs.v, MI30_N);
    sc_mul(u1, rn, m);
    sc_neg(u1, u1);
    sc_mul(u2, rn, ss);

    sc k1, k2;
    sc_split_lambda(k1, k2, u2);
    glv_make_odd(k1, k2);
    bool neg1 = sc_is_high(k1), neg2 = sc_is_high(k2);
    {
        sc nk;
        sc_neg(nk, k1);
#pragma unroll
        for (int i = 0; i < 8; i++) k1.v[i] = neg1 ? nk.v[i] : k1.v[i];
        sc_neg(nk, k2);
#pragma unroll
        for (int i = 0; i < 8; i++) k2.v[i] = neg2 ? nk.v[i] : k2.v[i];
    }
    uint32_t dig1[DIG_WORDS], dig2[DIG_WORDS], skew1, skew2;
    recode_glv(dig1, skew1, k1);
    recode_glv(dig2, skew2, k2);

    constexpr int PNT = GLV_NT - GLV_LNT;
    uint32_t ptab[18 * (PNT > 0 ? PNT : 1)];
#define GLV_L(i) ltab[(i) * GSV_LTAB_STRIDE]
#define GLV_X(e, k) ((e) < GLV_LNT ? GLV_L((e) * 9 + (k)) : ptab[((e) - GLV_LNT) * 9 + (k)])
#define GLV_Y(e, k) ((e) < GLV_LNT ? GLV_L(9 * GLV_LNT + (e) * 9 + (k)) : ptab[9 * PNT + ((e) - GLV_LNT) * 9 + (k)])
#define GLV_SET(e, k, X, Y)                                           \
    do {                                                              \
        if ((e) < GLV_LNT) {                                          \
            GLV_L((e) * 9 + (k)) = (X);                               \
            GLV_L(9 * GLV_LNT + (e) * 9 + (k)) = (Y);                 \
        } else {                                                      \
            ptab[((e) - GLV_LNT) * 9 + (k)] = (X);                    \
            ptab[9 * PNT + ((e) - GLV_LNT) * 9 + (k)] = (Y);          \
        }                                                             \
    } while (0)
    fe9 zfac;
    {
        ge9 Dp, P;
        fe9 zd;
        ge9_dblu(Dp, P, zd, x, y);
        fe9 zr[GLV_NT];
#pragma unroll
        for (int e = 0; e < GLV_NT; e++) {
            if (e) {
                ge9 Pn;
                ge9_zaddu(Pn, Dp, zr[e], P);
                P = Pn;
            }
#pragma unroll
            for (int k = 0; k < 9; k++) GLV_SET(e, k, P.x.v[k], P.y.v[k]);
        }
        fe9 f = zr[GLV_NT - 1];
#pragma unroll
        for (int e = GLV_NT - 2; e >= 0; e--) {
            fe9 ex, ey;
#pragma unroll
            for (int k = 0; k < 9; k++) {
                ex.v[k] = GLV_X(e, k);
                ey.v[k] = GLV_Y(e, k);
            }
            ge9 q;
            scale_xy9(q, ex, ey, f);
#pragma unroll
            for (int k = 0; k < 9; k++) GLV_SET(e, k, q.x.v[k], q.y.v[k]);
            if (e) fe9_mul(f, f, zr[e]);
        }
        fe9_mul(zfac, f, zd);
    }

    gej9 acc;
    bool ainf = true;
#pragma unroll
    for (int k = 0; k < 9; k++) {
        acc.x.v[k] = GLV_X(0, k);
        acc.y.v[k] = GLV_Y(0, k);
    }
    fe9_set_u32(acc.z, 1);
#pragma unroll 1
    for (int i = GLV_DIGITS - 1; i >= 0; i--) {
        if (i != GLV_DIGITS - 1) {
#pragma unroll 1
            for (int d = 0; d < GLV_W; d++) gej9_dbl(acc, acc);
        }
        constexpr uint32_t CMASK = (1u << DIG_SLOT) - 1u;
        uint32_t c1 = (sel_word(dig1, (uint32_t)i / DIG_PER_WORD) >> ((i % DIG_PER_WORD) * DIG_SLOT)) & CMASK;
        uint32_t c2 = (sel_word(dig2, (uint32_t)i / DIG_PER_WORD) >> ((i % DIG_PER_WORD) * DIG_SLOT)) & CMASK;
#pragma unroll 1
        for (int j = 0; j < 2; j++) {
            uint32_t c = j ? c2 : c1;
            bool ng = j ? neg2 : neg1;
            uint32_t ei = c & (uint32_t)(GLV_NT - 1);
            ge9 P;
            if (GLV_LNT == GLV_NT || (GLV_LNT > 0 && ei < (uint32_t)GLV_LNT)) {
                uint32_t xo = ei * 9u;
#pragma unroll
                for (int k = 0; k < 9; k++) {
                    P.x.v[k] = GLV_L(xo + k);
                    P.y.v[k] = GLV_L(9u * GLV_LNT + xo + k);
                }
            } else {
                uint32_t xo = (ei - (uint32_t)GLV_LNT) * 9u;
#pragma unroll
                for (int k = 0; k < 9; k++) {
                    P.x.v[k] = ptab[xo + k];
                    P.y.v[k] = ptab[9u * PNT + xo + k];
                }
            }
            if (j != 0) {
                fe9 beta;
                fe9_from_const(beta, BETA);
                fe9_mul(P.x, P.x, beta);
            }
            fe9 ny;
            fe9_neg<1>(ny, P.y);
            fe9_cmov(P.y, ny, ((c >> (GLV_W - 1)) != 0) != ng);
            if (i == GLV_DIGITS - 1 && j == 0) {
                acc.x = P.x;
                acc.y = P.y;
                fe9_normalize_weak(acc.y);
                fe9_set_u32(acc.z, 1);
                ainf = false;
                continue;
            }
            gej9_add_ge(acc, ainf, acc, P);
        }
    }
    fe9_mul(acc.z, acc.z, zfac);

    gej9 accg;
    bool ginf;
    comb_mul_g9(accg, ginf, u1, gtab);

    ok = recover_tail_twisted(qx, qy, accg, ginf, acc, ainf, c, recid & 1u) && ok;
    return ok ? GSV_ST_OK : GSV_ST_RECOVER_FAILED;
}

GSV_DI void load32_be(uint32_t v[8], const uint8_t* p) { limbs_from_be(v, p); }

GSV_DI void store_pub_addr(uint8_t* pub65, uint8_t* addr20, bool ok, const fe& qx, const fe& qy) {
    if (pub65) {
        pub65[0] = ok ? 4 : 0;
#pragma unroll
        for (int i = 0; i < 8; i++) {
            uint32_t xv = ok ? qx.v[7 - i] : 0u, yv = ok ? qy.v[7 - i] : 0u;
#pragma unroll
            for (int b = 0; b < 4; b++) {
                pub65[1 + 4 * i + b] = (uint8_t)(xv >> (24 - 8 * b));
                pub65[33 + 4 * i + b] = (uint8_t)(yv >> (24 - 8 * b));
            }
        }
    }
    if (addr20) {
        uint32_t h[8];
        keccak256_xy(h, qx.v, qy.v);
#pragma unroll
        for (int w = 3; w < 8; w++)
#pragma unroll
            for (int b = 0; b < 4; b++) addr20[(w - 3) * 4 + b] = ok ? (uint8_t)(h[w] >> (8 * b)) : 0;
    }
}


GSV_DI void derive32(uint32_t out_be_limbs[8], uint64_t seed, uint64_t i, uint32_t tag3) {
    uint64_t a[25];
#pragma unroll
    for (int k = 0; k < 25; k++) a[k] = 0;
    a[0] = seed;
    a[1] = i;
    a[2] = (uint64_t)(tag3 & 0xFFFFFFu) | (0x01ull << 24);
    a[16] = 0x8000000000000000ULL;
    keccakf(a);
#pragma unroll
    for (int j = 0; j < 4; j++) {
        out_be_limbs[7 - 2 * j] = __builtin_bswap32((uint32_t)a[j]);
        out_be_limbs[6 - 2 * j] = __builtin_bswap32((uint32_t)(a[j] >> 32));
    }
}

GSV_DI void ecdsa_sign(uint32_t r_out[8], uint32_t s_out[8], uint32_t& recid, fe& px, fe& py, sc d, sc k,
                       const uint32_t m[8], const uint4* __restrict__ gtab) {
    sc_cond_sub_n(d.v, d.v, 0);
    sc_cond_sub_n(k.v, k.v, 0);
    if (sc_is_zero(d)) d.v[0] = 1;
    if (sc_is_zero(k)) k.v[0] = 1;
    sc mr;
    sc_cond_sub_n(mr.v, m, 0);
    gej9 P;
    bool pinf;
    comb_mul_g9(P, pinf, d, gtab);
    gej9_to_affine_words(px, py, P);
    gej9 R;
    bool rinf;
    comb_mul_g9(R, rinf, k, gtab);
    fe rx, ry;
    gej9_to_affine_words(rx, ry, R);
    recid = ry.v[0] & 1u;
    sc r;
    bool over = !limbs_lt(rx.v, SN);
    sc_cond_sub_n(r.v, rx.v, 0);
    if (over) recid |= 2u;
    sc kinv, s, t;
    modinv30_words_ct(kinv.v, k.v, MI30_N);
    sc_mul(t, r, d);
    sc_add(t, t, mr);
    sc_mul(s, kinv, t);
    if (sc_is_high(s)) {
        sc_neg(s, s);
        recid ^= 1u;
    }
#pragma unroll
    for (int i = 0; i < 8; i++) {
        r_out[i] = r.v[i];
        s_out[i] = s.v[i];
    }
}

}
```

geth-sharding_amd/csrc/secp256k1_fe9.cuh:

```cuda
#pragma once
#include <stdint.h>

#include "opcount.cuh"

#if defined(__HIP_DEVICE_COMPILE__) && !defined(FE9_NO_ASM)
#include "fe9_asm.cuh"
#define FE9_ASM 1
#endif

#if defined(__HIPCC__)
#define FE9_FN __device__ __forceinline__
#define FE9_CONST __device__ constexpr
#else
#define FE9_FN static inline
#define FE9_CONST static constexpr
#endif

namespace gsv {

constexpr uint32_t M29 = 0x1FFFFFFFu;
constexpr uint32_t M24 = 0x00FFFFFFu;

struct fe9 { uint32_t v[9]; };

FE9_CONST uint32_t FE9_P[9] = {0x1FFFFC2Fu, 0x1FFFFFF7u, 0x1FFFFFFFu, 0x1FFFFFFFu, 0x1FFFFFFFu,
                               0x1FFFFFFFu, 0x1FFFFFFFu, 0x1FFFFFFFu, 0x00FFFFFFu};
FE9_CONST uint32_t FE9_Q[8][9] = {
    {0u, 0u, 0u, 0u, 0u, 0u, 0u, 0u, 0u},
#include "fe9_q_consts.inc"
};

FE9_FN void fe9_opaque(fe9& r) {
#if defined(__HIPCC__)
    asm volatile("" : "+v"(r.v[0]), "+v"(r.v[1]), "+v"(r.v[2]), "+v"(r.v[3]), "+v"(r.v[4]), "+v"(r.v[5]),
                 "+v"(r.v[6]), "+v"(r.v[7]), "+v"(r.v[8]));
#endif
}

FE9_FN void fe9_mac(uint64_t& acc, uint32_t a, uint32_t b) {
    acc += (uint64_t)a * b;
#if defined(FE9_ASM)
    asm("" : "+v"(acc));
#endif
}

FE9_FN void fe9_reduce(fe9& r, const uint32_t o[17], uint64_t o17) {
    uint32_t k256 = 256u;
#if defined(__HIPCC__) && !defined(FE9_NO_OPAQUE_256)
    asm("" : "+s"(k256));
#endif
    uint32_t carry = 0;
#pragma unroll
    for (int j = 0; j < 8; j++) {
        uint64_t c = (uint64_t)(o[j] + carry);
        fe9_mac(c, o[j + 9], 31264u);
        if (j) fe9_mac(c, o[j + 8], k256);
        r.v[j] = (uint32_t)c & M29;
        carry = (uint32_t)(c >> 29);
    }
    uint64_t c = (uint64_t)(o[8] + carry);
    c += o17 * 31264u;
    fe9_mac(c, o[16], k256);
    r.v[8] = (uint32_t)c & M24;
    uint64_t T = (c >> 24) + (o17 << 13);
    c = (uint64_t)r.v[0] + T * 977u;
    r.v[0] = (uint32_t)c & M29;
    c >>= 29;
    c += (uint64_t)r.v[1] + (T << 3);
    r.v[1] = (uint32_t)c & M29;
    c >>= 29;
    r.v[2] += (uint32_t)c;
    fe9_opaque(r);
}

FE9_FN void fe9_mul(fe9& r, const fe9& a, const fe9& b) {
    GSV_OPC(gsv::OPC_FE_MUL);
    uint32_t o[17];
#if defined(FE9_ASM)
    fe9_mul_full(r.v, a.v, b.v);
#else
    uint64_t acc = 0;
#pragma unroll
    for (int k = 0; k < 17; k++) {
#pragma unroll
        for (int i = 0; i < 9; i++) {
            int j = k - i;
            if (j >= 0 && j < 9) acc += (uint64_t)a.v[i] * b.v[j];
        }
        o[k] = (uint32_t)acc & M29;
        acc >>= 29;
    }
    fe9_reduce(r, o, acc);
#endif
}

FE9_FN void fe9_sqr(fe9& r, const fe9& a) {
    GSV_OPC(gsv::OPC_FE_SQR);
    uint32_t a2[9];
#pragma unroll
    for (int i = 0; i < 9; i++) a2[i] = a.v[i] << 1;
    uint32_t o[17];
#if defined(FE9_ASM)
    fe9_sqr_full(r.v, a.v, a2);
#else
    uint64_t acc = 0;
#pragma unroll
    for (int k = 0; k < 17; k++) {
#pragma unroll
        for (int i = 0; i < 9; i++) {
            int j = k - i;
            if (j > i && j < 9) acc += (uint64_t)a.v[i] * a2[j];
        }
        if ((k & 1) == 0 && k / 2 < 9) acc += (uint64_t)a.v[k / 2] * a.v[k / 2];
        o[k] = (uint32_t)acc & M29;
        acc >>= 29;
    }
    fe9_reduce(r, o, acc);
#endif
}

FE9_FN void fe9_mul_add(fe9& r, const fe9& a, const fe9& b, const fe9& c) {
    GSV_OPC(gsv::OPC_FE_MUL);
#if defined(FE9_ASM)
    fe9_mul_add_full(r.v, a.v, b.v, c.v);
#else
    uint32_t o[17];
    uint64_t acc = 0;
#pragma unroll
    for (int k = 0; k < 17; k++) {
#pragma unroll
        for (int i = 0; i < 9; i++) {
            int j = k - i;
            if (j >= 0 && j < 9) acc += (uint64_t)a.v[i] * b.v[j];
        }
        o[k] = (uint32_t)acc & M29;
        acc >>= 29;
    }
#pragma unroll
    for (int j = 0; j < 9; j++) o[j] += c.v[j];
    fe9_reduce(r, o, acc);
#endif
}
FE9_FN void fe9_dot(fe9& r, const fe9& a, const fe9& b, const fe9& c, const fe9& d) {
    GSV_OPC(gsv::OPC_FE_DOT);
#if defined(FE9_ASM)
    fe9_dot_full(r.v, a.v, b.v, c.v, d.v);
#else
    uint32_t o[17];
    uint64_t acc = 0;
#pragma unroll
    for (int k = 0; k < 17; k++) {
#pragma unroll
        for (int i = 0; i < 9; i++) {
            int j = k - i;
            if (j >= 0 && j < 9) acc += (uint64_t)a.v[i] * b.v[j] + (uint64_t)c.v[i] * d.v[j];
        }
        o[k] = (uint32_t)acc & M29;
        acc >>= 29;
    }
    fe9_reduce(r, o, acc);
#endif
}
FE9_FN void fe9_sqr_add(fe9& r, const fe9& a, const fe9& c) {
    GSV_OPC(gsv::OPC_FE_SQR);
    uint32_t a2[9];
#pragma unroll
    for (int i = 0; i < 9; i++) a2[i] = a.v[i] << 1;
#if defined(FE9_ASM)
    fe9_sqr_add_full(r.v, a.v, a2, c.v);
#else
    uint32_t o[17];
    uint64_t acc = 0;
#pragma unroll
    for (int k = 0; k < 17; k++) {
#pragma unroll
        for (int i = 0; i < 9; i++) {
            int j = k - i;
            if (j > i && j < 9) acc += (uint64_t)a.v[i] * a2[j];
        }
        if ((k & 1) == 0 && k / 2 < 9) acc += (uint64_t)a.v[k / 2] * a.v[k / 2];
        o[k] = (uint32_t)acc & M29;
        acc >>= 29;
    }
#pragma unroll
    for (int j = 0; j < 9; j++) o[j] += c.v[j];
    fe9_reduce(r, o, acc);
#endif
}

FE9_FN void fe9_sqr_n(fe9& r, const fe9& a, int n) {
    r = a;
    fe9 t;
#if defined(__HIPCC__)
#pragma unroll 1
#endif
    for (int i = 0; i + 1 < n; i += 2) {
        fe9_sqr(t, r);
        fe9_sqr(r, t);
    }
    if (n & 1) fe9_sqr(r, r);
}

FE9_FN void fe9_add(fe9& r, const fe9& a, const fe9& b) {
#pragma unroll
    for (int i = 0; i < 9; i++) r.v[i] = a.v[i] + b.v[i];
    fe9_opaque(r);
}
FE9_FN void fe9_mul_small(fe9& r, const fe9& a, uint32_t k) {
#pragma unroll
    for (int i = 0; i < 9; i++) r.v[i] = a.v[i] * k;
    fe9_opaque(r);
}
template <int M>
FE9_FN void fe9_sub(fe9& r, const fe9& a, const fe9& b) {
    static_assert(M >= 1 && M <= 7, "fe9_sub magnitude");
#pragma unroll
    for (int i = 0; i < 9; i++) r.v[i] = a.v[i] + (FE9_Q[M][i] - b.v[i]);
    fe9_opaque(r);
}
template <int M>
FE9_FN void fe9_negsum(fe9& c, const fe9& x, const fe9& y) {
    static_assert(M >= 1 && M <= 3, "fe9_negsum magnitude (addend limbs < 2^31)");
#pragma unroll
    for (int i = 0; i < 9; i++) c.v[i] = FE9_Q[M][i] - x.v[i] - y.v[i];
    fe9_opaque(c);
}
template <int M>
FE9_FN void fe9_negsum3(fe9& c, const fe9& x, const fe9& y, const fe9& z) {
    static_assert(M >= 1 && M <= 3, "fe9_negsum3 magnitude (addend limbs < 2^31)");
#pragma unroll
    for (int i = 0; i < 9; i++) c.v[i] = FE9_Q[M][i] - x.v[i] - y.v[i] - z.v[i];
    fe9_opaque(c);
}
template <int M>
FE9_FN void fe9_neg(fe9& r, const fe9& a) {
    static_assert(M >= 1 && M <= 7, "fe9_neg magnitude");
#pragma unroll
    for (int i = 0; i < 9; i++) r.v[i] = FE9_Q[M][i] - a.v[i];
    fe9_opaque(r);
}

FE9_FN void fe9_normalize_weak(fe9& r) {
    uint32_t c = 0;
#pragma unroll
    for (int i = 0; i < 8; i++) {
        uint32_t t = r.v[i] + c;
        r.v[i] = t & M29;
        c = t >> 29;
    }
    uint32_t t8 = r.v[8] + c;
    r.v[8] = t8 & M24;
    uint32_t T = t8 >> 24;
    uint32_t t0 = r.v[0] + T * 977u;
    r.v[0] = t0 & M29;
    uint32_t t1 = r.v[1] + (T << 3) + (t0 >> 29);
    r.v[1] = t1 & M29;
    r.v[2] += t1 >> 29;
    fe9_opaque(r);
}

FE9_FN void fe9_normalize_full(fe9& r) {
    fe9_normalize_weak(r);
    uint32_t c = 0;
#pragma unroll
    for (int i = 2; i < 8; i++) {
        uint32_t t = r.v[i] + c;
        r.v[i] = t & M29;
        c = t >> 29;
    }
    uint32_t t8 = r.v[8] + c;
    r.v[8] = t8 & M24;
    uint32_t T = t8 >> 24;
    uint32_t s[9];
    uint32_t t = r.v[0] + 977u;
    s[0] = t & M29;
    t = r.v[1] + 8u + (t >> 29);
    s[1] = t & M29;
#pragma unroll
    for (int i = 2; i < 8; i++) {
        t = r.v[i] + (t >> 29);
        s[i] = t & M29;
    }
    t = r.v[8] + (t >> 29);
    s[8] = t & M24;
    bool take = ((t >> 24) | T) != 0;
#pragma unroll
    for (int i = 0; i < 9; i++) r.v[i] = take ? s[i] : r.v[i];
    fe9_opaque(r);
}

FE9_FN bool fe9_is_zero_canon(const fe9& a) {
    uint32_t o = 0;
#pragma unroll
    for (int i = 0; i < 9; i++) o |= a.v[i];
    return o == 0;
}
FE9_FN bool fe9_is_zero(const fe9& a) {
    fe9 t = a;
    fe9_normalize_full(t);
    return fe9_is_zero_canon(t);
}
FE9_FN bool fe9_is_zero_weak(const fe9& a) {
    uint32_t z = 0, q = 0;
#pragma unroll
    for (int i = 0; i < 9; i++) {
        z |= a.v[i];
        q |= a.v[i] ^ FE9_P[i];
    }
    return z == 0 || q == 0;
}
FE9_FN bool fe9_eq_canon(const fe9& a, const fe9& b) {
    uint32_t o = 0;
#pragma unroll
    for (int i = 0; i < 9; i++) o |= a.v[i] ^ b.v[i];
    return o == 0;
}
FE9_FN void fe9_set_u32(fe9& r, uint32_t x) {
    r.v[0] = x;
#pragma unroll
    for (int i = 1; i < 9; i++) r.v[i] = 0;
}
FE9_FN void fe9_cmov(fe9& r, const fe9& a, bool flag) {
#pragma unroll
    for (int i = 0; i < 9; i++) r.v[i] = flag ? a.v[i] : r.v[i];
}

FE9_FN void fe9_from_words(fe9& r, const uint32_t w[8]) {
#pragma unroll
    for (int i = 0; i < 9; i++) {
        int bit = 29 * i, wi = bit >> 5, sh = bit & 31;
        uint32_t lo = w[wi] >> sh;
        uint32_t hi = (sh > 3 && wi + 1 < 8) ? (w[wi + 1] << (32 - sh)) : 0u;
        r.v[i] = (lo | hi) & M29;
    }
}
FE9_FN void fe9_to_words(uint32_t w[8], const fe9& a) {
#pragma unroll
    for (int j = 0; j < 8; j++) {
        int bit = 32 * j, li = bit / 29, sh = bit % 29;
        uint32_t x = a.v[li] >> sh;
        if (li + 1 < 9) x |= a.v[li + 1] << (29 - sh);
        if (sh > 26 && li + 2 < 9) x |= a.v[li + 2] << (58 - sh);
        w[j] = x;
    }
}

FE9_FN void fe9_pow_x223(fe9& x223, fe9& x22, fe9& x2, const fe9& a) {
    fe9 x3, x6, x9, x11, x44, x88, x176, x220, t;
    fe9_sqr(x2, a);
    fe9_mul(x2, x2, a);
    fe9_sqr(x3, x2);
    fe9_mul(x3, x3, a);
    fe9_sqr_n(t, x3, 3);
    fe9_mul(x6, t, x3);
    fe9_sqr_n(t, x6, 3);
    fe9_mul(x9, t, x3);
    fe9_sqr_n(t, x9, 2);
    fe9_mul(x11, t, x2);
    fe9_sqr_n(t, x11, 11);
    fe9_mul(x22, t, x11);
    fe9_sqr_n(t, x22, 22);
    fe9_mul(x44, t, x22);
    fe9_sqr_n(t, x44, 44);
    fe9_mul(x88, t, x44);
    fe9_sqr_n(t, x88, 88);
    fe9_mul(x176, t, x88);
    fe9_sqr_n(t, x176, 44);
    fe9_mul(x220, t, x44);
    fe9_sqr_n(t, x220, 3);
    fe9_mul(x223, t, x3);
}
FE9_FN void fe9_inv(fe9& r, const fe9& a) {
    fe9 x223, x22, x2, t;
    fe9_pow_x223(x223, x22, x2, a);
    fe9_sqr_n(t, x223, 23);
    fe9_mul(t, t, x22);
    fe9_sqr_n(t, t, 5);
    fe9_mul(t, t, a);
    fe9_sqr_n(t, t, 3);
    fe9_mul(t, t, x2);
    fe9_sqr_n(t, t, 2);
    fe9_mul(r, t, a);
}
FE9_FN bool fe9_sqrt(fe9& r, const fe9& a) {
    fe9 x223, x22, x2, t;
    fe9_pow_x223(x223, x22, x2, a);
    fe9_sqr_n(t, x223, 23);
    fe9_mul(t, t, x22);
    fe9_sqr_n(t, t, 6);
    fe9_mul(t, t, x2);
    fe9_sqr_n(r, t, 2);
    fe9_sqr(t, r);
    fe9_normalize_full(t);
    fe9 ac = a;
    fe9_normalize_full(ac);
    return fe9_eq_canon(t, ac);
}
FE9_FN void fe9_pow_pm3_4(fe9& r, const fe9& a) {
    fe9 x223, x22, x2, t;
    fe9_pow_x223(x223, x22, x2, a);
    fe9_sqr_n(t, x223, 23);
    fe9_mul(t, t, x22);
    fe9_sqr_n(t, t, 5);
    fe9_mul(t, t, a);
    fe9_sqr_n(t, t, 3);
    fe9_mul(r, t, x2);
}

struct gej9 { fe9 x, y, z; };
struct ge9 { fe9 x, y; };

FE9_FN void gej9_dbl(gej9& r, const gej9& p) {
    fe9 A, B, D, C4, E, F, t, u;
    fe9_sqr(A, p.x);
    fe9_sqr(B, p.y);
    fe9_mul_small(t, B, 4);
    fe9_mul(D, p.x, t);
    fe9_add(t, B, B);
    fe9_sqr(C4, t);
    fe9_mul_small(E, A, 3);
    fe9_normalize_weak(E);
    fe9 z2;
    fe9_add(z2, p.z, p.z);
    fe9_mul(r.z, p.y, z2);
    fe9_negsum<2>(t, D, D);
    fe9_sqr_add(u, E, t);
    fe9_sub<1>(t, D, u);
    fe9_negsum<2>(F, C4, C4);
    fe9_mul_add(r.y, E, t, F);
    r.x = u;
}

FE9_FN void gej9_add_ge_core(gej9& o, fe9& h, fe9& rr, const gej9& p, const ge9& q) {
    fe9 z1z1, s2, hh, i4, j, v, t;
    fe9_sqr(z1z1, p.z);
    fe9_neg<1>(t, p.x);
    fe9_mul_add(h, q.x, z1z1, t);
    fe9_mul(s2, q.y, p.z);
    fe9_add(s2, s2, s2);
    fe9_negsum<2>(t, p.y, p.y);
    fe9_mul_add(rr, s2, z1z1, t);
    fe9_sqr(hh, h);
    fe9_mul_small(i4, hh, 4);
    fe9_mul(j, h, i4);
    fe9_mul(v, p.x, i4);
    fe9_negsum3<3>(t, j, v, v);
    fe9_sqr_add(o.x, rr, t);
    fe9_sub<1>(t, v, o.x);
    fe9 w;
    fe9_negsum<2>(w, j, j);
    fe9_dot(o.y, rr, t, p.y, w);
    fe9_add(t, p.z, h);
    fe9_negsum<2>(w, z1z1, hh);
    fe9_sqr_add(o.z, t, w);
}

#ifndef GEJ9_DBL_RARE
#define GEJ9_DBL_RARE(o, p) gej9_dbl(o, p)
#endif

#if defined(__HIP_DEVICE_COMPILE__)
#define FE9_ANY(x) (__any(x) != 0)
#else
#define FE9_ANY(x) (x)
#endif
FE9_FN void gej9_cmov(gej9& r, const gej9& a, bool f) {
    fe9_cmov(r.x, a.x, f);
    fe9_cmov(r.y, a.y, f);
    fe9_cmov(r.z, a.z, f);
}
FE9_FN void gej9_add_ge(gej9& r, bool& inf, const gej9& p, const ge9& q) {
    gej9 o;
    fe9 h, rr;
    gej9_add_ge_core(o, h, rr, p, q);
    bool exc = !inf && fe9_is_zero_weak(h);
    if (FE9_ANY(exc || inf)) {
        bool dbl = exc && fe9_is_zero(rr);
        bool neg = exc && !dbl;
        if (FE9_ANY(dbl)) {
            gej9 d;
            GEJ9_DBL_RARE(d, p);
            gej9_cmov(o, d, dbl);
        }
        gej9_cmov(o, p, neg);
        if (FE9_ANY(inf)) {
            gej9 qn;
            qn.x = q.x;
            qn.y = q.y;
            fe9_normalize_weak(qn.x);
            fe9_normalize_weak(qn.y);
            fe9_set_u32(qn.z, 1);
            gej9_cmov(o, qn, inf);
        }
        inf = neg;
    } else {
        inf = false;
    }
    r = o;
}

FE9_FN void gej9_add(gej9& r, bool& rinf, const gej9& p, bool pinf, const gej9& q, bool qinf) {
    if (pinf) { r = q; rinf = qinf; return; }
    if (qinf) { r = p; rinf = false; return; }
    fe9 z1z1, z2z2, u1, u2, s1, s2, h, rr, i, j, v, t, w;
    fe9_sqr(z1z1, p.z);
    fe9_sqr(z2z2, q.z);
    fe9_mul(u1, p.x, z2z2);
    fe9_mul(u2, q.x, z1z1);
    fe9_mul(s1, p.y, q.z);
    fe9_mul(s1, s1, z2z2);
    fe9_mul(s2, q.y, p.z);
    fe9_mul(s2, s2, z1z1);
    fe9_sub<1>(h, u2, u1);
    fe9_normalize_weak(h);
    fe9_sub<1>(rr, s2, s1);
    fe9_normalize_weak(rr);
    if (fe9_is_zero_weak(h)) {
        if (fe9_is_zero_weak(rr)) {
            gej9_dbl(r, p);
            rinf = false;
        } else {
            rinf = true;
            r = p;
        }
        return;
    }
    fe9_add(t, h, h);
    fe9_sqr(i, t);
    fe9_mul(j, h, i);
    fe9_add(rr, rr, rr);
    fe9_mul(v, u1, i);
    gej9 o;
    fe9_sqr(t, rr);
    fe9_sub<1>(t, t, j);
    fe9_add(w, v, v);
    fe9_sub<2>(t, t, w);
    fe9_normalize_weak(t);
    o.x = t;
    fe9_sub<1>(t, v, o.x);
    fe9_mul(t, rr, t);
    fe9_mul(w, s1, j);
    fe9_add(w, w, w);
    fe9_sub<2>(t, t, w);
    fe9_normalize_weak(t);
    o.y = t;
    fe9_mul(t, p.z, q.z);
    fe9_mul(t, t, h);
    fe9_add(o.z, t, t);
    r = o;
    rinf = false;
}

FE9_FN void gej9_add_ge_zr(gej9& r, fe9& zr, const gej9& p, const ge9& q) {
    fe9 h, rr;
    gej9_add_ge_core(r, h, rr, p, q);
    fe9_add(zr, h, h);
}


FE9_FN void ge9_dblu(ge9& d, ge9& rp, fe9& z, const fe9& x, const fe9& y) {
    fe9 A, B, t, C4, E, u;
    fe9_sqr(A, x);
    fe9_sqr(B, y);
    fe9_mul_small(t, B, 4);
    fe9_mul(rp.x, x, t);
    fe9_add(t, B, B);
    fe9_sqr(C4, t);
    fe9_mul_small(E, A, 3);
    fe9_normalize_weak(E);
    fe9_add(z, y, y);
    fe9_negsum<2>(t, rp.x, rp.x);
    fe9_sqr_add(d.x, E, t);
    fe9_sub<1>(u, rp.x, d.x);
    fe9_negsum<2>(t, C4, C4);
    fe9_mul_add(d.y, E, u, t);
    fe9_add(rp.y, C4, C4);
    fe9_normalize_weak(rp.y);
}

FE9_FN void ge9_zaddu(ge9& s, ge9& p1, fe9& zr, const ge9& p2) {
    fe9 C, W1, W2, rr, t, u, A1;
    fe9_sub<1>(zr, p1.x, p2.x);
    fe9_normalize_weak(zr);
    fe9_sqr(C, zr);
    fe9_mul(W1, p1.x, C);
    fe9_mul(W2, p2.x, C);
    fe9_sub<1>(rr, p1.y, p2.y);
    fe9_normalize_weak(rr);
    fe9_negsum<2>(t, W1, W2);
    fe9_sqr_add(s.x, rr, t);
    fe9_sub<1>(t, W1, W2);
    fe9_mul(A1, p1.y, t);
    fe9_sub<1>(u, W1, s.x);
    fe9_neg<1>(t, A1);
    fe9_mul_add(s.y, rr, u, t);
    p1.x = W1;
    p1.y = A1;
}

FE9_FN void scale_xy9(ge9& r, const fe9& x, const fe9& y, const fe9& f) {
    fe9 f2, f3;
    fe9_sqr(f2, f);
    fe9_mul(f3, f2, f);
    fe9_mul(r.x, x, f2);
    fe9_mul(r.y, y, f3);
}

FE9_FN void build_r_table9(ge9 T[4], fe9& zfac, const fe9& x, const fe9& y) {
    ge9 Dp, P1, P3, P5, P7;
    fe9 zd, zr3, zr5, zr7;
    ge9_dblu(Dp, P1, zd, x, y);
    ge9_zaddu(P3, Dp, zr3, P1);
    ge9_zaddu(P5, Dp, zr5, P3);
    ge9_zaddu(P7, Dp, zr7, P5);
    T[3] = P7;
    scale_xy9(T[2], P5.x, P5.y, zr7);
    fe9 f;
    fe9_mul(f, zr5, zr7);
    scale_xy9(T[1], P3.x, P3.y, f);
    fe9_mul(f, f, zr3);
    scale_xy9(T[0], P1.x, P1.y, f);
    fe9_mul(f, f, zd);
    zfac = f;
}

}
```

Baseline: 119.7 million sigs/s.

## Use scaled Jacobian coordinates with fused dot/square kernels for GLV ladder

Switches the GLV double-and-add loop and the G comb to a scaled Jacobian representation (y doubled, later rescaled) whose doubling formula needs fewer field operations. It adds fused asm primitives: a*b+c^2 and 3a^2, with negating doublings that cancel out in pairs (hence the even-window assertion). A conversion back to standard Jacobian runs once at the end. The aim is to cut multiplies and reductions per doubling and addition, at the cost of new inline asm and added correctness risk in the exceptional cases.

Measured after the change: 124.9 million sigs/s (median of 6 runs). 1.04x the previous value.

```diff
diff --git a/geth-sharding_amd/csrc/fe9_asm.cuh b/geth-sharding_amd/csrc/fe9_asm.cuh
--- a/geth-sharding_amd/csrc/fe9_asm.cuh
+++ b/geth-sharding_amd/csrc/fe9_asm.cuh
@@ -41,4 +41,20 @@
         : "v"(a[0]), "v"(a[1]), "v"(a[2]), "v"(a[3]), "v"(a[4]), "v"(a[5]), "v"(a[6]), "v"(a[7]), "v"(a[8]), "v"(b[0]), "v"(b[1]), "v"(b[2]), "v"(b[3]), "v"(b[4]), "v"(b[5]), "v"(b[6]), "v"(b[7]), "v"(b[8]), "s"(k31264), "s"(k256), "s"(k977), "s"(k8192), "v"(c[0]), "v"(c[1]), "v"(c[2]), "v"(c[3]), "v"(c[4]), "v"(c[5]), "v"(c[6]), "v"(c[7]), "v"(c[8]), "v"(d[0]), "v"(d[1]), "v"(d[2]), "v"(d[3]), "v"(d[4]), "v"(d[5]), "v"(d[6]), "v"(d[7]), "v"(d[8])
         : "v2", "v3", "v4", "v5", "v6", "v7", "v8", "v9", "v10", "v11", "v12", "v13", "v14", "v15", "v16", "v17", "v18", "v19");
 }
+__device__ __forceinline__ void fe9_dot_ms_full(uint32_t r[9], const uint32_t a[9], const uint32_t b[9], const uint32_t c[9], const uint32_t d[9]) {
+    uint64_t sd;
+    uint32_t k31264 = 31264u, k256 = 256u, k977 = 977u, k8192 = 8192u;
+    asm("v_mad_u64_u32 v[2:3], %9, %11, %27, 0\n\tv_mad_u64_u32 v[2:3], %9, %12, %26, v[2:3]\n\tv_mad_u64_u32 v[2:3], %9, %13, %25, v[2:3]\n\tv_mad_u64_u32 v[2:3], %9, %14, %24, v[2:3]\n\tv_mad_u64_u32 v[2:3], %9, %15, %23, v[2:3]\n\tv_mad_u64_u32 v[2:3], %9, %16, %22, v[2:3]\n\tv_mad_u64_u32 v[2:3], %9, %17, %21, v[2:3]\n\tv_mad_u64_u32 v[2:3], %9, %18, %20, v[2:3]\n\tv_mad_u64_u32 v[2:3], %9, %33, %49, v[2:3]\n\tv_mad_u64_u32 v[2:3], %9, %34, %48, v[2:3]\n\tv_mad_u64_u32 v[2:3], %9, %35, %47, v[2:3]\n\tv_mad_u64_u32 v[2:3], %9, %36, %46, v[2:3]\n\tv_mad_u64_u32 v[6:7], %9, v3, 8, 0\n\tv_mad_u64_u32 v[6:7], %9, %12, %27, v[6:7]\n\tv_mad_u64_u32 v[6:7], %9, %13, %26, v[6:7]\n\tv_mad_u64_u32 v[6:7], %9, %14, %25, v[6:7]\n\tv_mad_u64_u32 v[6:7], %9, %15, %24, v[6:7]\n\tv_mad_u64_u32 v[6:7], %9, %16, %23, v[6:7]\n\tv_mad_u64_u32 v[6:7], %9, %17, %22, v[6:7]\n\tv_mad_u64_u32 v[6:7], %9, %18, %21, v[6:7]\n\tv_mad_u64_u32 v[6:7], %9, %34, %49, v[6:7]\n\tv_mad_u64_u32 v[6:7], %9, %35, %48, v[6:7]\n\tv_mad_u64_u32 v[6:7], %9, %36, %47, v[6:7]\n\tv_mad_u64_u32 v[6:7], %9, %37, %37, v[6:7]\n\tv_mad_u64_u32 v[8:9], %9, v7, 8, 0\n\tv_mad_u64_u32 v[8:9], %9, %13, %27, v[8:9]\n\tv_mad_u64_u32 v[8:9], %9, %14, %26, v[8:9]\n\tv_mad_u64_u32 v[8:9], %9, %15, %25, v[8:9]\n\tv_mad_u64_u32 v[8:9], %9, %16, %24, v[8:9]\n\tv_mad_u64_u32 v[8:9], %9, %17, %23, v[8:9]\n\tv_mad_u64_u32 v[8:9], %9, %18, %22, v[8:9]\n\tv_mad_u64_u32 v[8:9], %9, %35, %49, v[8:9]\n\tv_mad_u64_u32 v[8:9], %9, %36, %48, v[8:9]\n\tv_mad_u64_u32 v[8:9], %9, %37, %47, v[8:9]\n\tv_mad_u64_u32 v[10:11], %9, v9, 8, 0\n\tv_mad_u64_u32 v[10:11], %9, %14, %27, v[10:11]\n\tv_mad_u64_u32 v[10:11], %9, %15, %26, v[10:11]\n\tv_mad_u64_u32 v[10:11], %9, %16, %25, v[10:11]\n\tv_mad_u64_u32 v[10:11], %9, %17, %24, v[10:11]\n\tv_mad_u64_u32 v[10:11], %9, %18, %23, v[10:11]\n\tv_mad_u64_u32 v[10:11], %9, %36, %49, v[10:11]\n\tv_mad_u64_u32 v[10:11], %9, %37, %48, v[10:11]\n\tv_mad_u64_u32 v[10:11], %9, %38, %38, v[10:11]\n\tv_mad_u64_u32 v[12:13], %9, v11, 8, 0\n\tv_mad_u64_u32 v[12:13], %9, %15, %27, v[12:13]\n\tv_mad_u64_u32 v[12:13], %9, %16, %26, v[12:13]\n\tv_mad_u64_u32 v[12:13], %9, %17, %25, v[12:13]\n\tv_mad_u64_u32 v[12:13], %9, %18, %24, v[12:13]\n\tv_mad_u64_u32 v[12:13], %9, %37, %49, v[12:13]\n\tv_mad_u64_u32 v[12:13], %9, %38, %48, v[12:13]\n\tv_mad_u64_u32 v[14:15], %9, v13, 8, 0\n\tv_mad_u64_u32 v[14:15], %9, %16, %27, v[14:15]\n\tv_mad_u64_u32 v[14:15], %9, %17, %26, v[14:15]\n\tv_mad_u64_u32 v[14:15], %9, %18, %25, v[14:15]\n\tv_mad_u64_u32 v[14:15], %9, %38, %49, v[14:15]\n\tv_mad_u64_u32 v[14:15], %9, %39, %39, v[14:15]\n\tv_mad_u64_u32 v[16:17], %9, v15, 8, 0\n\tv_mad_u64_u32 v[16:17], %9, %17, %27, v[16:17]\n\tv_mad_u64_u32 v[16:17], %9, %18, %26, v[16:17]\n\tv_mad_u64_u32 v[16:17], %9, %39, %49, v[16:17]\n\tv_mad_u64_u32 v[18:19], %9, v17, 8, 0\n\tv_mad_u64_u32 v[18:19], %9, %18, %27, v[18:19]\n\tv_mad_u64_u32 v[18:19], %9, %40, %40, v[18:19]\n\tv_lshlrev_b32 v3, 3, v19\n\tv_mad_u64_u32 v[4:5], %9, %10, %19, 0\n\tv_mad_u64_u32 v[4:5], %9, %32, %32, v[4:5]\n\tv_mad_u64_u32 v[4:5], %9, v2, %28, v[4:5]\n\tv_and_b32_e32 %0, 0x1fffffff, v4\n\tv_lshrrev_b64 v[4:5], 29, v[4:5]\n\tv_mad_u64_u32 v[4:5], %9, %10, %20, v[4:5]\n\tv_mad_u64_u32 v[4:5], %9, %11, %19, v[4:5]\n\tv_mad_u64_u32 v[4:5], %9, %32, %42, v[4:5]\n\tv_mad_u64_u32 v[4:5], %9, v6, %28, v[4:5]\n\tv_mad_u64_u32 v[4:5], %9, v2, %29, v[4:5]\n\tv_and_b32_e32 %1, 0x1fffffff, v4\n\tv_lshrrev_b64 v[4:5], 29, v[4:5]\n\tv_mad_u64_u32 v[4:5], %9, %10, %21, v[4:5]\n\tv_mad_u64_u32 v[4:5], %9, %11, %20, v[4:5]\n\tv_mad_u64_u32 v[4:5], %9, %12, %19, v[4:5]\n\tv_mad_u64_u32 v[4:5], %9, %32, %43, v[4:5]\n\tv_mad_u64_u32 v[4:5], %9, %33, %33, v[4:5]\n\tv_mad_u64_u32 v[4:5], %9, v8, %28, v[4:5]\n\tv_mad_u64_u32 v[4:5], %9, v6, %29, v[4:5]\n\tv_and_b32_e32 %2, 0x1fffffff, v4\n\tv_lshrrev_b64 v[4:5], 29, v[4:5]\n\tv_mad_u64_u32 v[4:5], %9, %10, %22, v[4:5]\n\tv_mad_u64_u32 v[4:5], %9, %11, %21, v[4:5]\n\tv_mad_u64_u32 v[4:5], %9, %12, %20, v[4:5]\n\tv_mad_u64_u32 v[4:5], %9, %13, %19, v[4:5]\n\tv_mad_u64_u32 v[4:5], %9, %32, %44, v[4:5]\n\tv_mad_u64_u32 v[4:5], %9, %33, %43, v[4:5]\n\tv_mad_u64_u32 v[4:5], %9, v10, %28, v[4:5]\n\tv_mad_u64_u32 v[4:5], %9, v8, %29, v[4:5]\n\tv_and_b32_e32 %3, 0x1fffffff, v4\n\tv_lshrrev_b64 v[4:5], 29, v[4:5]\n\tv_mad_u64_u32 v[4:5], %9, %10, %23, v[4:5]\n\tv_mad_u64_u32 v[4:5], %9, %11, %22, v[4:5]\n\tv_mad_u64_u32 v[4:5], %9, %12, %21, v[4:5]\n\tv_mad_u64_u32 v[4:5], %9, %13, %20, v[4:5]\n\tv_mad_u64_u32 v[4:5], %9, %14, %19, v[4:5]\n\tv_mad_u64_u32 v[4:5], %9, %32, %45, v[4:5]\n\tv_mad_u64_u32 v[4:5], %9, %33, %44, v[4:5]\n\tv_mad_u64_u32 v[4:5], %9, %34, %34, v[4:5]\n\tv_mad_u64_u32 v[4:5], %9, v12, %28, v[4:5]\n\tv_mad_u64_u32 v[4:5], %9, v10, %29, v[4:5]\n\tv_and_b32_e32 %4, 0x1fffffff, v4\n\tv_lshrrev_b64 v[4:5], 29, v[4:5]\n\tv_mad_u64_u32 v[4:5], %9, %10, %24, v[4:5]\n\tv_mad_u64_u32 v[4:5], %9, %11, %23, v[4:5]\n\tv_mad_u64_u32 v[4:5], %9, %12, %22, v[4:5]\n\tv_mad_u64_u32 v[4:5], %9, %13, %21, v[4:5]\n\tv_mad_u64_u32 v[4:5], %9, %14, %20, v[4:5]\n\tv_mad_u64_u32 v[4:5], %9, %15, %19, v[4:5]\n\tv_mad_u64_u32 v[4:5], %9, %32, %46, v[4:5]\n\tv_mad_u64_u32 v[4:5], %9, %33, %45, v[4:5]\n\tv_mad_u64_u32 v[4:5], %9, %34, %44, v[4:5]\n\tv_mad_u64_u32 v[4:5], %9, v14, %28, v[4:5]\n\tv_mad_u64_u32 v[4:5], %9, v12, %29, v[4:5]\n\tv_and_b32_e32 %5, 0x1fffffff, v4\n\tv_lshrrev_b64 v[4:5], 29, v[4:5]\n\tv_mad_u64_u32 v[4:5], %9, %10, %25, v[4:5]\n\tv_mad_u64_u32 v[4:5], %9, %11, %24, v[4:5]\n\tv_mad_u64_u32 v[4:5], %9, %12, %23, v[4:5]\n\tv_mad_u64_u32 v[4:5], %9, %13, %22, v[4:5]\n\tv_mad_u64_u32 v[4:5], %9, %14, %21, v[4:5]\n\tv_mad_u64_u32 v[4:5], %9, %15, %20, v[4:5]\n\tv_mad_u64_u32 v[4:5], %9, %16, %19, v[4:5]\n\tv_mad_u64_u32 v[4:5], %9, %32, %47, v[4:5]\n\tv_mad_u64_u32 v[4:5], %9, %33, %46, v[4:5]\n\tv_mad_u64_u32 v[4:5], %9, %34, %45, v[4:5]\n\tv_mad_u64_u32 v[4:5], %9, %35, %35, v[4:5]\n\tv_mad_u64_u32 v[4:5], %9, v16, %28, v[4:5]\n\tv_mad_u64_u32 v[4:5], %9, v14, %29, v[4:5]\n\tv_and_b32_e32 %6, 0x1fffffff, v4\n\tv_lshrrev_b64 v[4:5], 29, v[4:5]\n\tv_mad_u64_u32 v[4:5], %9, %10, %26, v[4:5]\n\tv_mad_u64_u32 v[4:5], %9, %11, %25, v[4:5]\n\tv_mad_u64_u32 v[4:5], %9, %12, %24, v[4:5]\n\tv_mad_u64_u32 v[4:5], %9, %13, %23, v[4:5]\n\tv_mad_u64_u32 v[4:5], %9, %14, %22, v[4:5]\n\tv_mad_u64_u32 v[4:5], %9, %15, %21, v[4:5]\n\tv_mad_u64_u32 v[4:5], %9, %16, %20, v[4:5]\n\tv_mad_u64_u32 v[4:5], %9, %17, %19, v[4:5]\n\tv_mad_u64_u32 v[4:5], %9, %32, %48, v[4:5]\n\tv_mad_u64_u32 v[4:5], %9, %33, %47, v[4:5]\n\tv_mad_u64_u32 v[4:5], %9, %34, %46, v[4:5]\n\tv_mad_u64_u32 v[4:5], %9, %35, %45, v[4:5]\n\tv_mad_u64_u32 v[4:5], %9, v18, %28, v[4:5]\n\tv_mad_u64_u32 v[4:5], %9, v16, %29, v[4:5]\n\tv_and_b32_e32 %7, 0x1fffffff, v4\n\tv_lshrrev_b64 v[4:5], 29, v[4:5]\n\tv_mad_u64_u32 v[4:5], %9, %10, %27, v[4:5]\n\tv_mad_u64_u32 v[4:5], %9, %11, %26, v[4:5]\n\tv_mad_u64_u32 v[4:5], %9, %12, %25, v[4:5]\n\tv_mad_u64_u32 v[4:5], %9, %13, %24, v[4:5]\n\tv_mad_u64_u32 v[4:5], %9, %14, %23, v[4:5]\n\tv_mad_u64_u32 v[4:5], %9, %15, %22, v[4:5]\n\tv_mad_u64_u32 v[4:5], %9, %16, %21, v[4:5]\n\tv_mad_u64_u32 v[4:5], %9, %17, %20, v[4:5]\n\tv_mad_u64_u32 v[4:5], %9, %18, %19, v[4:5]\n\tv_mad_u64_u32 v[4:5], %9, %32, %49, v[4:5]\n\tv_mad_u64_u32 v[4:5], %9, %33, %48, v[4:5]\n\tv_mad_u64_u32 v[4:5], %9, %34, %47, v[4:5]\n\tv_mad_u64_u32 v[4:5], %9, %35, %46, v[4:5]\n\tv_mad_u64_u32 v[4:5], %9, %36, %36, v[4:5]\n\tv_mad_u64_u32 v[4:5], %9, v3, %28, v[4:5]\n\tv_mad_u64_u32 v[4:5], %9, v18, %29, v[4:5]\n\tv_and_b32_e32 %8, 0xffffff, v4\n\tv_lshrrev_b64 v[4:5], 24, v[4:5]\n\tv_mad_u64_u32 v[6:7], %9, v3, %31, v[4:5]\n\tv_mov_b32 v5, 0\n\tv_mov_b32 v4, %0\n\tv_mad_u64_u32 v[4:5], %9, v6, %30, v[4:5]\n\tv_mad_u32_u24 v5, v7, %30, v5\n\tv_and_b32_e32 %0, 0x1fffffff, v4\n\tv_lshrrev_b64 v[4:5], 29, v[4:5]\n\tv_lshl_add_u64 v[4:5], v[6:7], 3, v[4:5]\n\tv_mad_u64_u32 v[4:5], %9, %1, 1, v[4:5]\n\tv_and_b32_e32 %1, 0x1fffffff, v4\n\tv_alignbit_b32 v6, v5, v4, 29\n\tv_add_u32 %2, %2, v6"
+        : "=&v"(r[0]), "=&v"(r[1]), "=&v"(r[2]), "=&v"(r[3]), "=&v"(r[4]), "=&v"(r[5]), "=&v"(r[6]), "=&v"(r[7]), "=&v"(r[8]), "=&s"(sd)
+        : "v"(a[0]), "v"(a[1]), "v"(a[2]), "v"(a[3]), "v"(a[4]), "v"(a[5]), "v"(a[6]), "v"(a[7]), "v"(a[8]), "v"(b[0]), "v"(b[1]), "v"(b[2]), "v"(b[3]), "v"(b[4]), "v"(b[5]), "v"(b[6]), "v"(b[7]), "v"(b[8]), "s"(k31264), "s"(k256), "s"(k977), "s"(k8192), "v"(c[0]), "v"(c[1]), "v"(c[2]), "v"(c[3]), "v"(c[4]), "v"(c[5]), "v"(c[6]), "v"(c[7]), "v"(c[8]), "v"(d[0]), "v"(d[1]), "v"(d[2]), "v"(d[3]), "v"(d[4]), "v"(d[5]), "v"(d[6]), "v"(d[7]), "v"(d[8])
+        : "v2", "v3", "v4", "v5", "v6", "v7", "v8", "v9", "v10", "v11", "v12", "v13", "v14", "v15", "v16", "v17", "v18", "v19");
 }
+__device__ __forceinline__ void fe9_sqr3_full(uint32_t r[9], const uint32_t a[9], const uint32_t b[9], const uint32_t c[9]) {
+    uint64_t sd;
+    uint32_t k31264 = 31264u, k256 = 256u, k977 = 977u, k8192 = 8192u;
+    asm("v_mad_u64_u32 v[2:3], %9, %11, %27, 0\n\tv_mad_u64_u32 v[2:3], %9, %12, %26, v[2:3]\n\tv_mad_u64_u32 v[2:3], %9, %13, %25, v[2:3]\n\tv_mad_u64_u32 v[2:3], %9, %14, %24, v[2:3]\n\tv_mad_u64_u32 v[6:7], %9, v3, 8, 0\n\tv_mad_u64_u32 v[6:7], %9, %12, %27, v[6:7]\n\tv_mad_u64_u32 v[6:7], %9, %13, %26, v[6:7]\n\tv_mad_u64_u32 v[6:7], %9, %14, %25, v[6:7]\n\tv_mad_u64_u32 v[6:7], %9, %15, %37, v[6:7]\n\tv_mad_u64_u32 v[8:9], %9, v7, 8, 0\n\tv_mad_u64_u32 v[8:9], %9, %13, %27, v[8:9]\n\tv_mad_u64_u32 v[8:9], %9, %14, %26, v[8:9]\n\tv_mad_u64_u32 v[8:9], %9, %15, %25, v[8:9]\n\tv_mad_u64_u32 v[10:11], %9, v9, 8, 0\n\tv_mad_u64_u32 v[10:11], %9, %14, %27, v[10:11]\n\tv_mad_u64_u32 v[10:11], %9, %15, %26, v[10:11]\n\tv_mad_u64_u32 v[10:11], %9, %16, %38, v[10:11]\n\tv_mad_u64_u32 v[12:13], %9, v11, 8, 0\n\tv_mad_u64_u32 v[12:13], %9, %15, %27, v[12:13]\n\tv_mad_u64_u32 v[12:13], %9, %16, %26, v[12:13]\n\tv_mad_u64_u32 v[14:15], %9, v13, 8, 0\n\tv_mad_u64_u32 v[14:15], %9, %16, %27, v[14:15]\n\tv_mad_u64_u32 v[14:15], %9, %17, %39, v[14:15]\n\tv_mad_u64_u32 v[16:17], %9, v15, 8, 0\n\tv_mad_u64_u32 v[16:17], %9, %17, %27, v[16:17]\n\tv_mad_u64_u32 v[18:19], %9, v17, 8, 0\n\tv_mad_u64_u32 v[18:19], %9, %18, %40, v[18:19]\n\tv_lshlrev_b32 v3, 3, v19\n\tv_mad_u64_u32 v[4:5], %9, %10, %32, 0\n\tv_mad_u64_u32 v[4:5], %9, v2, %28, v[4:5]\n\tv_and_b32_e32 %0, 0x1fffffff, v4\n\tv_lshrrev_b64 v[4:5], 29, v[4:5]\n\tv_mad_u64_u32 v[4:5], %9, %10, %20, v[4:5]\n\tv_mad_u64_u32 v[4:5], %9, v6, %28, v[4:5]\n\tv_mad_u64_u32 v[4:5], %9, v2, %29, v[4:5]\n\tv_and_b32_e32 %1, 0x1fffffff, v4\n\tv_lshrrev_b64 v[4:5], 29, v[4:5]\n\tv_mad_u64_u32 v[4:5], %9, %10, %21, v[4:5]\n\tv_mad_u64_u32 v[4:5], %9, %11, %33, v[4:5]\n\tv_mad_u64_u32 v[4:5], %9, v8, %28, v[4:5]\n\tv_mad_u64_u32 v[4:5], %9, v6, %29, v[4:5]\n\tv_and_b32_e32 %2, 0x1fffffff, v4\n\tv_lshrrev_b64 v[4:5], 29, v[4:5]\n\tv_mad_u64_u32 v[4:5], %9, %10, %22, v[4:5]\n\tv_mad_u64_u32 v[4:5], %9, %11, %21, v[4:5]\n\tv_mad_u64_u32 v[4:5], %9, v10, %28, v[4:5]\n\tv_mad_u64_u32 v[4:5], %9, v8, %29, v[4:5]\n\tv_and_b32_e32 %3, 0x1fffffff, v4\n\tv_lshrrev_b64 v[4:5], 29, v[4:5]\n\tv_mad_u64_u32 v[4:5], %9, %10, %23, v[4:5]\n\tv_mad_u64_u32 v[4:5], %9, %11, %22, v[4:5]\n\tv_mad_u64_u32 v[4:5], %9, %12, %34, v[4:5]\n\tv_mad_u64_u32 v[4:5], %9, v12, %28, v[4:5]\n\tv_mad_u64_u32 v[4:5], %9, v10, %29, v[4:5]\n\tv_and_b32_e32 %4, 0x1fffffff, v4\n\tv_lshrrev_b64 v[4:5], 29, v[4:5]\n\tv_mad_u64_u32 v[4:5], %9, %10, %24, v[4:5]\n\tv_mad_u64_u32 v[4:5], %9, %11, %23, v[4:5]\n\tv_mad_u64_u32 v[4:5], %9, %12, %22, v[4:5]\n\tv_mad_u64_u32 v[4:5], %9, v14, %28, v[4:5]\n\tv_mad_u64_u32 v[4:5], %9, v12, %29, v[4:5]\n\tv_and_b32_e32 %5, 0x1fffffff, v4\n\tv_lshrrev_b64 v[4:5], 29, v[4:5]\n\tv_mad_u64_u32 v[4:5], %9, %10, %25, v[4:5]\n\tv_mad_u64_u32 v[4:5], %9, %11, %24, v[4:5]\n\tv_mad_u64_u32 v[4:5], %9, %12, %23, v[4:5]\n\tv_mad_u64_u32 v[4:5], %9, %13, %35, v[4:5]\n\tv_mad_u64_u32 v[4:5], %9, v16, %28, v[4:5]\n\tv_mad_u64_u32 v[4:5], %9, v14, %29, v[4:5]\n\tv_and_b32_e32 %6, 0x1fffffff, v4\n\tv_lshrrev_b64 v[4:5], 29, v[4:5]\n\tv_mad_u64_u32 v[4:5], %9, %10, %26, v[4:5]\n\tv_mad_u64_u32 v[4:5], %9, %11, %25, v[4:5]\n\tv_mad_u64_u32 v[4:5], %9, %12, %24, v[4:5]\n\tv_mad_u64_u32 v[4:5], %9, %13, %23, v[4:5]\n\tv_mad_u64_u32 v[4:5], %9, v18, %28, v[4:5]\n\tv_mad_u64_u32 v[4:5], %9, v16, %29, v[4:5]\n\tv_and_b32_e32 %7, 0x1fffffff, v4\n\tv_lshrrev_b64 v[4:5], 29, v[4:5]\n\tv_mad_u64_u32 v[4:5], %9, %10, %27, v[4:5]\n\tv_mad_u64_u32 v[4:5], %9, %11, %26, v[4:5]\n\tv_mad_u64_u32 v[4:5], %9, %12, %25, v[4:5]\n\tv_mad_u64_u32 v[4:5], %9, %13, %24, v[4:5]\n\tv_mad_u64_u32 v[4:5], %9, %14, %36, v[4:5]\n\tv_mad_u64_u32 v[4:5], %9, v3, %28, v[4:5]\n\tv_mad_u64_u32 v[4:5], %9, v18, %29, v[4:5]\n\tv_and_b32_e32 %8, 0xffffff, v4\n\tv_lshrrev_b64 v[4:5], 24, v[4:5]\n\tv_mad_u64_u32 v[6:7], %9, v3, %31, v[4:5]\n\tv_mov_b32 v5, 0\n\tv_mov_b32 v4, %0\n\tv_mad_u64_u32 v[4:5], %9, v6, %30, v[4:5]\n\tv_mad_u32_u24 v5, v7, %30, v5\n\tv_and_b32_e32 %0, 0x1fffffff, v4\n\tv_lshrrev_b64 v[4:5], 29, v[4:5]\n\tv_lshl_add_u64 v[4:5], v[6:7], 3, v[4:5]\n\tv_mad_u64_u32 v[4:5], %9, %1, 1, v[4:5]\n\tv_and_b32_e32 %1, 0x1fffffff, v4\n\tv_alignbit_b32 v6, v5, v4, 29\n\tv_add_u32 %2, %2, v6"
+        : "=&v"(r[0]), "=&v"(r[1]), "=&v"(r[2]), "=&v"(r[3]), "=&v"(r[4]), "=&v"(r[5]), "=&v"(r[6]), "=&v"(r[7]), "=&v"(r[8]), "=&s"(sd)
+        : "v"(a[0]), "v"(a[1]), "v"(a[2]), "v"(a[3]), "v"(a[4]), "v"(a[5]), "v"(a[6]), "v"(a[7]), "v"(a[8]), "v"(b[0]), "v"(b[1]), "v"(b[2]), "v"(b[3]), "v"(b[4]), "v"(b[5]), "v"(b[6]), "v"(b[7]), "v"(b[8]), "s"(k31264), "s"(k256), "s"(k977), "s"(k8192), "v"(c[0]), "v"(c[1]), "v"(c[2]), "v"(c[3]), "v"(c[4]), "v"(c[5]), "v"(c[6]), "v"(c[7]), "v"(c[8])
+        : "v2", "v3", "v4", "v5", "v6", "v7", "v8", "v9", "v10", "v11", "v12", "v13", "v14", "v15", "v16", "v17", "v18", "v19");
+}
+}
diff --git a/geth-sharding_amd/csrc/opcount.cuh b/geth-sharding_amd/csrc/opcount.cuh
--- a/geth-sharding_amd/csrc/opcount.cuh
+++ b/geth-sharding_amd/csrc/opcount.cuh
@@ -10,7 +10,8 @@
     OPC_MODINV = 5,
     OPC_BN_REDC = 6,
     OPC_FE_DOT = 7,
-    OPC_N = 8
+    OPC_FE_DOT_MS = 8,
+    OPC_N = 9
 };
 }
 
diff --git a/geth-sharding_amd/csrc/recover_dev.cuh b/geth-sharding_amd/csrc/recover_dev.cuh
--- a/geth-sharding_amd/csrc/recover_dev.cuh
+++ b/geth-sharding_amd/csrc/recover_dev.cuh
@@ -2,8 +2,13 @@
 #include "gsv_internal.h"
 #include "keccak_dev.cuh"
 #include "secp256k1_dev.cuh"
-namespace gsv { struct gej9; __device__ void gej9_dbl_rare(gej9& o, const gej9& p); }
+namespace gsv {
+struct gej9;
+__device__ void gej9_dbl_rare(gej9& o, const gej9& p);
+__device__ void gejw_dbl_rare(gej9& o, const gej9& p);
+}
 #define GEJ9_DBL_RARE(o, p) gej9_dbl_rare(o, p)
+#define GEJW_DBL_RARE(o, p) gejw_dbl_rare(o, p)
 #include "secp256k1_fe9.cuh"
 #include "modinv30.cuh"
 
@@ -31,6 +36,7 @@
                                            0xFFFFFFFFu, 0xFFFFFFFFu, 0xFFFFFFFFu, 0x7FFFFFFFu};
 
 constexpr int GLV_W = 4;
+static_assert(GLV_W % 2 == 0, "an odd run of negating doublings leaves the accumulator at -2^W P");
 constexpr int GLV_NT = 1 << (GLV_W - 1);
 constexpr int GLV_DIGITS = (130 + GLV_W - 1) / GLV_W;
 constexpr int DIG_SLOT = GLV_W <= 4 ? 4 : 8;
@@ -133,6 +139,7 @@
 }
 
 typedef uint32_t gsv_v32 __attribute__((ext_vector_type(32)));
+template <bool WCONV>
 __device__ __noinline__ gsv_v32 gej9_dbl_ool(gsv_v32 in) {
     gej9 p, d;
 #pragma unroll
@@ -141,7 +148,8 @@
         p.y.v[i] = in[9 + i];
         p.z.v[i] = in[18 + i];
     }
-    gej9_dbl(d, p);
+    if (WCONV) gejw_dbl(d, p);
+    else gej9_dbl(d, p);
     gsv_v32 o;
 #pragma unroll
     for (int i = 0; i < 9; i++) {
@@ -153,7 +161,8 @@
     for (int i = 27; i < 32; i++) o[i] = 0;
     return o;
 }
-__device__ void gej9_dbl_rare(gej9& o, const gej9& p) {
+template <bool WCONV>
+GSV_DI void gej9_dbl_rare_call(gej9& o, const gej9& p) {
     gsv_v32 in;
 #pragma unroll
     for (int i = 0; i < 9; i++) {
@@ -163,7 +172,7 @@
     }
 #pragma unroll
     for (int i = 27; i < 32; i++) in[i] = 0;
-    gsv_v32 d = gej9_dbl_ool(in);
+    gsv_v32 d = gej9_dbl_ool<WCONV>(in);
 #pragma unroll
     for (int i = 0; i < 9; i++) {
         o.x.v[i] = d[i];
@@ -171,6 +180,8 @@
         o.z.v[i] = d[18 + i];
     }
 }
+__device__ void gej9_dbl_rare(gej9& o, const gej9& p) { gej9_dbl_rare_call<false>(o, p); }
+__device__ void gejw_dbl_rare(gej9& o, const gej9& p) { gej9_dbl_rare_call<true>(o, p); }
 
 GSV_DI void table_select9(ge9& out, const ge9 T[4], uint32_t idx) {
     out = T[0];
@@ -207,7 +218,7 @@
     const uint32_t d0 = c[0] & MASK;
     gtab_load(Pn, gtab + (size_t)d0 * GTAB_ENTRY_U4);
     acc.x = Pn.x;
-    acc.y = Pn.y;
+    fe9_add(acc.y, Pn.y, Pn.y);
     fe9_set_u32(acc.z, 1);
     inf = d0 == 0;
     comb_shift(c);
@@ -222,12 +233,13 @@
         }
         gej9 t;
         bool tinf = inf;
-        gej9_add_ge(t, tinf, acc, P);
+        gejw_add_ge(t, tinf, acc, P);
         if (d != 0) {
             acc = t;
             inf = tinf;
         }
     }
+    gejw_to_gej9(acc, acc);
 }
 
 GSV_DI void gej9_to_affine_words(fe& ax, fe& ay, const gej9& q) {
@@ -501,7 +513,7 @@
     for (int i = GLV_DIGITS - 1; i >= 0; i--) {
         if (i != GLV_DIGITS - 1) {
 #pragma unroll 1
-            for (int d = 0; d < GLV_W; d++) gej9_dbl(acc, acc);
+            for (int d = 0; d < GLV_W; d++) gejw_dbl_neg(acc, acc);
         }
         constexpr uint32_t CMASK = (1u << DIG_SLOT) - 1u;
         uint32_t c1 = (sel_word(dig1, (uint32_t)i / DIG_PER_WORD) >> ((i % DIG_PER_WORD) * DIG_SLOT)) & CMASK;
@@ -537,15 +549,16 @@
             fe9_cmov(P.y, ny, ((c >> (GLV_W - 1)) != 0) != ng);
             if (i == GLV_DIGITS - 1 && j == 0) {
                 acc.x = P.x;
-                acc.y = P.y;
+                fe9_add(acc.y, P.y, P.y);
                 fe9_normalize_weak(acc.y);
                 fe9_set_u32(acc.z, 1);
                 ainf = false;
                 continue;
             }
-            gej9_add_ge(acc, ainf, acc, P);
-        }
-    }
+            gejw_add_ge(acc, ainf, acc, P);
+        }
+    }
+    gejw_to_gej9(acc, acc);
     fe9_mul(acc.z, acc.z, zfac);
 
     gej9 accg;
diff --git a/geth-sharding_amd/csrc/secp256k1_fe9.cuh b/geth-sharding_amd/csrc/secp256k1_fe9.cuh
--- a/geth-sharding_amd/csrc/secp256k1_fe9.cuh
+++ b/geth-sharding_amd/csrc/secp256k1_fe9.cuh
@@ -155,6 +155,62 @@
             int j = k - i;
             if (j >= 0 && j < 9) acc += (uint64_t)a.v[i] * b.v[j] + (uint64_t)c.v[i] * d.v[j];
         }
+        o[k] = (uint32_t)acc & M29;
+        acc >>= 29;
+    }
+    fe9_reduce(r, o, acc);
+#endif
+}
+FE9_FN void fe9_dot_ms(fe9& r, const fe9& a, const fe9& b, const fe9& c) {
+    GSV_OPC(gsv::OPC_FE_DOT_MS);
+    uint32_t c2[9];
+#pragma unroll
+    for (int i = 0; i < 9; i++) c2[i] = c.v[i] << 1;
+#if defined(FE9_ASM)
+    fe9_dot_ms_full(r.v, a.v, b.v, c.v, c2);
+#else
+    uint32_t o[17];
+    uint64_t acc = 0;
+#pragma unroll
+    for (int k = 0; k < 17; k++) {
+#pragma unroll
+        for (int i = 0; i < 9; i++) {
+            int j = k - i;
+            if (j >= 0 && j < 9) acc += (uint64_t)a.v[i] * b.v[j];
+            if (j > i && j < 9) acc += (uint64_t)c.v[i] * c2[j];
+        }
+        if ((k & 1) == 0 && k / 2 < 9) acc += (uint64_t)c.v[k / 2] * c.v[k / 2];
+        o[k] = (uint32_t)acc & M29;
+        acc >>= 29;
+    }
+    fe9_reduce(r, o, acc);
+#endif
+}
+FE9_FN void fe9_sqr3(fe9& r, const fe9& a) {
+    GSV_OPC(gsv::OPC_FE_SQR);
+    uint32_t a3[9], a6[9];
+#pragma unroll
+    for (int i = 0; i < 9; i++) {
+#if defined(FE9_ASM)
+        asm("v_lshl_add_u32 %0, %1, 1, %1" : "=v"(a3[i]) : "v"(a.v[i]));
+#else
+        a3[i] = (a.v[i] << 1) + a.v[i];
+#endif
+        a6[i] = a3[i] << 1;
+    }
+#if defined(FE9_ASM)
+    fe9_sqr3_full(r.v, a.v, a6, a3);
+#else
+    uint32_t o[17];
+    uint64_t acc = 0;
+#pragma unroll
+    for (int k = 0; k < 17; k++) {
+#pragma unroll
+        for (int i = 0; i < 9; i++) {
+            int j = k - i;
+            if (j > i && j < 9) acc += (uint64_t)a.v[i] * a6[j];
+        }
+        if ((k & 1) == 0 && k / 2 < 9) acc += (uint64_t)a.v[k / 2] * a3[k / 2];
         o[k] = (uint32_t)acc & M29;
         acc >>= 29;
     }
@@ -499,6 +555,93 @@
     r = o;
 }
 
+FE9_FN void gejw_dbl_neg(gej9& r, const gej9& p) {
+    fe9 B, D, E, t, u;
+    fe9_sqr3(E, p.x);
+    fe9_sqr(B, p.y);
+    fe9_mul(D, p.x, B);
+    fe9_mul(r.z, p.y, p.z);
+    fe9_negsum<2>(t, D, D);
+    fe9_sqr_add(u, E, t);
+    fe9_sub<1>(t, u, D);
+    fe9_add(t, t, t);
+    fe9_dot_ms(r.y, E, t, B);
+    r.x = u;
+}
+
+FE9_FN void gejw_add_ge_core(gej9& o, fe9& h, fe9& rr, const gej9& p, const ge9& q) {
+    fe9 z1z1, s2, hh, i4, j, v, t;
+    fe9_sqr(z1z1, p.z);
+    fe9_neg<1>(t, p.x);
+    fe9_mul_add(h, q.x, z1z1, t);
+    fe9_mul(s2, q.y, p.z);
+    fe9_add(s2, s2, s2);
+    fe9_neg<2>(t, p.y);
+    fe9_mul_add(rr, s2, z1z1, t);
+    fe9_sqr(hh, h);
+    fe9_mul_small(i4, hh, 4);
+    fe9_mul(j, h, i4);
+    fe9_mul(v, p.x, i4);
+    fe9_negsum3<3>(t, j, v, v);
+    fe9_sqr_add(o.x, rr, t);
+    fe9_sub<1>(t, v, o.x);
+    fe9 w;
+    fe9_neg<1>(w, j);
+    fe9_dot(o.y, rr, t, p.y, w);
+    fe9_add(o.y, o.y, o.y);
+    fe9_add(t, p.z, h);
+    fe9_negsum<2>(w, z1z1, hh);
+    fe9_sqr_add(o.z, t, w);
+}
+
+FE9_FN void gejw_dbl(gej9& r, const gej9& p) {
+    gejw_dbl_neg(r, p);
+    fe9_neg<1>(r.y, r.y);
+}
+#ifndef GEJW_DBL_RARE
+#define GEJW_DBL_RARE(o, p) gejw_dbl(o, p)
+#endif
+
+FE9_FN void gejw_add_ge(gej9& r, bool& inf, const gej9& p, const ge9& q) {
+    gej9 o;
+    fe9 h, rr;
+    gejw_add_ge_core(o, h, rr, p, q);
+    bool exc = !inf && fe9_is_zero_weak(h);
+    if (FE9_ANY(exc || inf)) {
+        bool dbl = exc && fe9_is_zero(rr);
+        bool neg = exc && !dbl;
+        if (FE9_ANY(dbl)) {
+            gej9 d;
+            GEJW_DBL_RARE(d, p);
+            gej9_cmov(o, d, dbl);
+        }
+        gej9_cmov(o, p, neg);
+        if (FE9_ANY(inf)) {
+            gej9 qn;
+            qn.x = q.x;
+            fe9_add(qn.y, q.y, q.y);
+            fe9_normalize_weak(qn.x);
+            fe9_normalize_weak(qn.y);
+            fe9_set_u32(qn.z, 1);
+            gej9_cmov(o, qn, inf);
+        }
+        inf = neg;
+    } else {
+        inf = false;
+    }
+    r = o;
+}
+
+FE9_FN void gejw_to_gej9(gej9& r, const gej9& p) {
+    fe9 w = p.y;
+    fe9_normalize_weak(w);
+    fe9_mul_small(r.x, p.x, 4);
+    fe9_normalize_weak(r.x);
+    fe9_mul_small(r.y, w, 4);
+    fe9_normalize_weak(r.y);
+    fe9_add(r.z, p.z, p.z);
+}
+
 FE9_FN void gej9_add(gej9& r, bool& rinf, const gej9& p, bool pinf, const gej9& q, bool qinf) {
     if (pinf) { r = q; rinf = qinf; return; }
     if (qinf) { r = p; rinf = false; return; }
```
